# JiawangBian/SC-SfMLearner-Release

Measured on NVIDIA H100. Metric: train-step frames/sec at 256x832 ResNet18 (DispResNet18+PoseResNet18, fwd+bwd+losses+Adam), higher is better.
Workload: dtype tf32x3 (3xTF32 split-accumulate, fp32-level)

## Files before the change

include/scsfm.h:

```cpp
#ifndef SCSFM_H_
#define SCSFM_H_

#include <stddef.h>
#include <stdint.h>

#ifdef __cplusplus
extern "C" {
#endif

#define SCSFM_OK 0
#define SCSFM_ERR_ARG (-1)
#define SCSFM_ERR_CUDA (-2)

#define SCSFM_MAX_JOBS 16

#define SCSFM_WITH_SSIM 1
#define SCSFM_WITH_MASK 2
#define SCSFM_WITH_AUTO_MASK 4
#define SCSFM_DEFER_FINALIZE 0x100
#define SCSFM_PAD_ZEROS 0
#define SCSFM_PAD_BORDER 1

const char* scsfm_last_error(void);
int scsfm_version(void);
long long scsfm_launch_count(void);

typedef struct ScsfmPairJob {
    const float* tgt_img;
    const float* ref_img;
    const float* tgt_depth;
    const float* ref_depth;
    const float* pose;
    float* grad_tgt_depth;
    float* grad_ref_depth;
    float* grad_pose;
    int tgt_shift;
    int ref_shift;
} ScsfmPairJob;

typedef struct ScsfmPairMaps {
    float* warped;
    float* valid;
    float* proj_depth;
    float* comp_depth;
    float* mask;
    float* diff_img;
    float* diff_depth;
} ScsfmPairMaps;

size_t scsfm_pairwise_stats_bytes(int njobs, int B);

int scsfm_pairwise_fwd(const ScsfmPairJob* jobs_host, int njobs, const float* intrinsics, int B, int H, int W,
                       int flags, int padding_mode, void* stats, float* loss_out, const ScsfmPairMaps* maps_host,
                       void* stream);

int scsfm_pairwise_finalize(void* stats, int njobs, float grad_scale, float* loss_out, void* stream);
int scsfm_pairwise_sums_count(int njobs);

int scsfm_pairwise_bwd(const ScsfmPairJob* jobs_host, int njobs, const float* intrinsics, int B, int H, int W,
                       int flags, int padding_mode, void* stats, const float* grad_out, void* stream);

int scsfm_inverse_warp2_fwd(const float* img, const float* depth, const float* ref_depth, const float* pose,
                            const float* intrinsics, int B, int H, int W, int padding_mode, float* warped,
                            float* valid, float* proj_depth, float* comp_depth, void* stream);

int scsfm_inverse_warp2_bwd(const float* img, const float* depth, const float* ref_depth, const float* pose,
                            const float* intrinsics, int B, int H, int W, int padding_mode,
                            const float* grad_warped, const float* grad_proj_depth, const float* grad_comp_depth,
                            float* grad_depth, float* grad_ref_depth, float* grad_pose, void* scratch_12B_doubles,
                            void* stream);

int scsfm_pose_vec2mat(const float* vec, int B, int rotation_mode, float* out, void* stream);

typedef struct ScsfmSmoothJob {
    const float* depth;
    const float* img;
    float* grad_depth;
} ScsfmSmoothJob;

size_t scsfm_smooth_stats_bytes(int njobs, int B);

int scsfm_smooth_fwd(const ScsfmSmoothJob* jobs_host, int njobs, int B, int H, int W, void* stats, float* loss_out,
                     void* stream);
int scsfm_smooth_bwd(const ScsfmSmoothJob* jobs_host, int njobs, int B, int H, int W, void* stats,
                     const float* grad_out, void* stream);


#define SCSFM_PADMODE_ZERO 0
#define SCSFM_PADMODE_REFLECT 1
#define SCSFM_ACT_NONE 0
#define SCSFM_ACT_RELU 1
#define SCSFM_ACT_ELU 2
#define SCSFM_ACT_DISP 3
#define SCSFM_BN_SLOTS 16
#define SCSFM_ROUND_TF32 0x100

typedef struct ScsfmConv {
    const float* in;
    const float* w;
    const float* bias;
    float* out;
    const float* dout;
    float* din;
    const float* addend;
    float* dw;
    float* dbias;
    double* bn_sums;
    int bn_groups;
    int B, Hi, Wi, Cin, Ho, Wo, Cout, kh, kw, stride, pad, pad_mode, act;
    const float* in_lo;
    const float* w_lo;
    const float* dout_lo;
    unsigned tune;
    unsigned long long* debug;
    const float* bn_scale;
    const float* bn_shift;
    float* out_lo;
} ScsfmConv;

#define SCSFM_TUNE_NO_TMA 0x1u
#define SCSFM_TUNE_MT(mt) (((unsigned)(mt) & 3u) << 4)
#define SCSFM_TUNE_TW(l2) (((unsigned)((l2) ? (l2) - 2 : 0) & 3u) << 6)
#define SCSFM_TUNE_BN(bn) (((bn) == 16 ? 1u : (bn) == 32 ? 2u : (bn) == 64 ? 3u : (bn) == 128 ? 4u : 0u) << 8)
#define SCSFM_TUNE_WGRAD(k) (((unsigned)(k) & 3u) << 12)

int scsfm_conv2d_fwd_simt(const ScsfmConv* p, void* stream);
int scsfm_conv2d_dgrad_simt(const ScsfmConv* p, void* stream);
int scsfm_conv2d_wgrad_simt(const ScsfmConv* p, void* stream);

int scsfm_conv2d_fwd_tc(const ScsfmConv* p, void* stream);
int scsfm_conv2d_dgrad_tc(const ScsfmConv* p, void* stream);
int scsfm_conv2d_wgrad_tc(const ScsfmConv* p, void* stream);
#define SCSFM_OPERAND_TF32 0
#define SCSFM_OPERAND_RAW 1
#define SCSFM_OPERAND_LO 2
int scsfm_weight_flip(const float* w, int Cout, int kh, int kw, int Cin, float* wt, int operand, void* stream);
int scsfm_weight_flip_s2(const float* w, int Cout, int kh, int kw, int Cin, int pad, float* wt4, int operand, void* stream);

int scsfm_weight_flip_batched(const long long* table, int n_rows, int total_blocks, void* stream);

int scsfm_head_conv_fwd(const float* in, const float* w, const float* bias, float* out, int B, int H, int W, int C, int act, void* stream);
int scsfm_head_conv_wgrad(const float* in, const float* dpre, float* dw, float* dbias, int B, int H, int W, int C, void* stream);
int scsfm_head_conv_dgrad(const float* dpre, const float* w, float* dpad, int B, int H, int W, int C, void* stream);

int scsfm_nchw_to_nhwc(const float* a, const float* b, int B, int C, int H, int W, float* out, void* stream);
int scsfm_nchw_to_nhwc_pad(const float* a, const float* b, int B, int C, int H, int W, int Cpad, float* out, int operand, void* stream);
int scsfm_pad_channels(const float* src, long long rows, int C, int Cpad, float* dst, int operand, void* stream);
int scsfm_unpad_add(const float* src, long long rows, int C, int Cpad, float* dst, void* stream);
int scsfm_nhwc_to_nchw(const float* in, int B, int C, int H, int W, float* out, void* stream);
int scsfm_stem_dgrad(const float* dy, const float* w, int N, int H, int W, int Cin, float* dimg1, float* dimg2, void* stream);

int scsfm_bn_prepare(const double* sums, int groups, int C, long long count_per_group, const float* gamma,
                     const float* beta, float* running_mean, float* running_var, float momentum, float eps,
                     int training, float* saved, void* stream);
int scsfm_bn_apply(const float* y, const double* sums, const float* gamma, const float* beta, float* running_mean,
                   float* running_var, float momentum, float eps, float* saved, const float* residual, float* z, float* z_lo,
                   long long rows, int C, int groups, int flags, void* stream);
int scsfm_bn_eval_prepare_batched(const long long* table, int n_layers, void* stream);
#define SCSFM_BN_FROZEN 0x200
int scsfm_bn_backward(const float* dz, const float* z, const float* y, const float* saved, const float* gamma,
                      float* dy, float* dy_lo, float* dres, float* dgamma, float* dbeta, long long rows, int C, int groups,
                      int relu, double* work, void* stream);

int scsfm_maxpool_fwd(const float* x, int B, int H, int W, int C, float* y, unsigned char* idx, void* stream);
int scsfm_maxpool_bwd(const float* dy, const unsigned char* idx, int B, int H, int W, int C, float* dx, int accumulate,
                      void* stream);

int scsfm_upcat_fwd(const float* lo, const float* skip, int B, int H, int W, int C1, int C2, float* out, void* stream);
int scsfm_fold_bwd(const float* dpad, int B, int H, int W, int C1, int C2, int upsample, float* d_lo,
                   const float* lo_act, int act, int accumulate, float* d_skip, void* stream);

int scsfm_act_bwd(float* d, const float* out, long long n, int act, void* stream);

int scsfm_spatial_mean_fwd(const float* x, int B, int HW, int C, float scale, float* out, void* stream);
int scsfm_spatial_mean_bwd(const float* dout, int B, int HW, int C, float scale, float* dx, void* stream);

int scsfm_compute_errors(const float* gt, const float* pred, int B, int H, int W, int y1, int y2, int x1, int x2,
                         float max_depth, void* work, float* out, void* stream);

#define SCSFM_EVAL_GT_F32 0
#define SCSFM_EVAL_GT_F64 1
#define SCSFM_EVAL_OUT 12
typedef struct ScsfmEvalDepthImage {
    long long gt_offset;
    int H, W;
    int y1, y2, x1, x2;
} ScsfmEvalDepthImage;
size_t scsfm_eval_depth_workspace_bytes(const ScsfmEvalDepthImage* images_host, int n_img);
int scsfm_eval_depth(const double* pred, int n_img, int h, int w, const void* gt, int gt_dtype, long long gt_elems,
                     const ScsfmEvalDepthImage* images_host, double min_depth, double max_depth, void* workspace,
                     size_t workspace_bytes, double* out, void* stream);

long long scsfm_augment_workspace_ints(int B, int H, int W);
int scsfm_augment_batch(const unsigned char* images, const int* params, int n_img, int B, int H, int W, const float* mean3,
                        const float* std3, float* out, int* workspace, long long workspace_ints, void* stream);

size_t scsfm_resize_bilinear_workspace_bytes(int B, int H, int W, int out_h, int out_w);
int scsfm_resize_bilinear_u8(const unsigned char* in, int B, int H, int W, int out_h, int out_w, unsigned char* out,
                             void* workspace, size_t workspace_bytes, void* stream);

size_t scsfm_velo_depth_workspace_bytes(int B, int Hd, int Wd);
int scsfm_velo_depth(const float* points, const long long* offsets, const long long* offsets_host, const double* P, int B,
                     int Hd, int Wd, float* depth, void* workspace, size_t workspace_bytes, void* stream);

int scsfm_round_tf32(const float* in, float* out, long long n, void* stream);
int scsfm_split_tf32(const float* in, float* lo, long long n, void* stream);

int scsfm_adam_step(float* param, const float* grad, float* exp_avg, float* exp_avg_sq, long long n, float lr,
                    float beta1, float beta2, float eps, float weight_decay, int step, const int* step_dev,
                    float* mirror, int mirror_operand, void* stream);

#ifdef __cplusplus
}
#endif
#endif
```

sc-sfmlearner-release_b200/csrc/conv_tc.cu:

```cuda
#include <stdlib.h>

#include "conv_tc.cuh"

namespace scsfm {

template <int BN, int STAGES, int A_BYTES, int B_BYTES>
__device__ __forceinline__ void gather_consume(float (&acc)[BN / 2], uint8_t* sA, uint8_t* sB, uint64_t* bar_full, uint64_t* bar_empty,
                                               int total, int chain) {
    float part[BN / 2];
#pragma unroll
    for (int i = 0; i < BN / 2; ++i) acc[i] = 0.f;
    for (int it0 = 0; it0 < total; it0 += chain) {
        const int it1 = min(total, it0 + chain);
        for (int it = it0; it < it1; ++it) {
            const int s = it % STAGES;
            tc::mbar_wait(bar_full + s, (it / STAGES) & 1);
            tc::fence_proxy_async();
            const uint32_t a_addr = tc::smem_u32(sA + s * A_BYTES), b_addr = tc::smem_u32(sB + s * B_BYTES);
            tc::reg_fence(part);
            tc::wgmma_fence();
#pragma unroll
            for (int j = 0; j < TBK / 8; ++j)
                tc::wgmma_tf32<BN>(part, tc::make_desc_sw128(a_addr + j * 32), tc::make_desc_sw128(b_addr + j * 32), (it == it0 && j == 0) ? 0u : 1u);
            tc::wgmma_commit();
            tc::wgmma_wait<1>();
            if (it > it0) tc::mbar_arrive(bar_empty + (it - 1) % STAGES);
        }
        tc::wgmma_wait<0>();
        tc::reg_fence(part);
        tc::mbar_arrive(bar_empty + (it1 - 1) % STAGES);
#pragma unroll
        for (int i = 0; i < BN / 2; ++i) acc[i] += part[i];
    }
}

template <int BN, bool STACK = false>
__global__ void __launch_bounds__(FW_THREADS)
conv_fwd_tc_kernel(ScsfmConv p, TcView v, const __grid_constant__ CUtensorMap wmap, const __grid_constant__ CUtensorMap wmap_lo) {
    using Cfg = TcCfg<BN>;
    constexpr int STAGES = Cfg::STAGES;
    extern __shared__ uint8_t smem_raw[];
    uint8_t* smem = reinterpret_cast<uint8_t*>((reinterpret_cast<uintptr_t>(smem_raw) + 1023) & ~uintptr_t(1023));
    uint8_t* sA = smem;
    uint8_t* sB = smem + STAGES * A_STAGE_BYTES;
    uint64_t* bar_full = reinterpret_cast<uint64_t*>(smem + (Cfg::OPERANDS > Cfg::EPI ? Cfg::OPERANDS : Cfg::EPI));
    uint64_t* bar_empty = bar_full + STAGES;

    const int tid = threadIdx.x, warp = tid >> 5, lane = tid & 31;
    const int rows_per_img = v.border ? border_count(p.Ho, p.Wo) : p.Ho * p.Wo;
    const int M = p.B * rows_per_img, N = p.Cout, K = v.kh * v.kw * p.Cin;
    const int m0 = blockIdx.x * GBM, n0 = blockIdx.y * BN;
    const int KB = (K + TBK - 1) / TBK;
    const int npass = STACK ? 2 : 1 + (p.in_lo != nullptr ? 1 : 0) + (p.w_lo != nullptr ? 1 : 0);
    const int chain = npass > 1 ? CHAIN_KB : KB * npass;

    if (tid == 0) {
        for (int s = 0; s < STAGES; ++s) {
            tc::mbar_init(bar_full + s, FW_PWARPS * 32 + 1);
            tc::mbar_init(bar_empty + s, 128);
        }
        tc::fence_barrier_init();
        tc::tma_prefetch_desc(&wmap);
        if (p.w_lo != nullptr) tc::tma_prefetch_desc(&wmap_lo);
    }
    __syncthreads();
    float acc[BN / 2];

    if (warp < FW_PWARPS) {
        constexpr int ROWS = GBM / (FW_PWARPS * 4);
        const int c = tid & 7;
        const int r0 = tid >> 3;
        const int cs = c ^ (r0 & 7);
        const bool reflect = p.pad_mode == PADMODE_REFLECT;
        int hi0[ROWS], wi0[ROWS], rbase[ROWS];
#pragma unroll
        for (int i = 0; i < ROWS; ++i) {
            const int m = m0 + r0 + 16 * i;
            if (m < M) {
                const int b = m / rows_per_img, rem = m - b * rows_per_img;
                int ho, wo;
                if (v.border) border_pixel(rem, p.Ho, p.Wo, ho, wo);
                else { ho = rem / p.Wo; wo = rem - ho * p.Wo; }
                hi0[i] = ho * v.in_stride + v.oy0;
                wi0[i] = wo * v.in_stride + v.ox0;
                rbase[i] = b * p.Hi * p.Wi * p.Cin;
            } else {
                hi0[i] = -(1 << 28);
                wi0[i] = -(1 << 28);
                rbase[i] = 0;
            }
        }
        const uint32_t a_smem = tc::smem_u32(sA) + (uint32_t)(r0 * 128 + cs * 16);
        const uint32_t b_smem = tc::smem_u32(sB);
        int kc, dy, dx, ch;
        int aoff[ROWS];
        uint32_t okm = 0;
        int it = 0;
        for (int q = 0; q < npass; ++q) {
        const int ps = (q + 1) % npass;
        const float* a_base = (ps == 1 && p.in_lo != nullptr) ? p.in_lo : p.in;
        const CUtensorMap* wm = (ps == npass - 1 && ps > 0 && p.w_lo != nullptr) ? &wmap_lo : &wmap;
        kc = 4 * c;
        {
            const int tap = kc / p.Cin;
            ch = kc - tap * p.Cin;
            dy = tap / v.kw;
            dx = tap - dy * v.kw;
        }
        int cur_dy = -1, cur_dx = -1;
        for (int kb = 0; kb < KB; ++kb, ++it) {
            const int s = it % STAGES;
            const uint32_t ph = (it / STAGES) & 1;
            if (lane == 0) tc::mbar_wait(bar_empty + s, ph ^ 1);
            __syncwarp();
            const uint32_t a_st = a_smem + (uint32_t)(s * A_STAGE_BYTES);
            if (tid == 0) {
                tc::mbar_arrive_expect_tx(bar_full + s, (uint32_t)Cfg::B_STAGE_BYTES);
                if (STACK) {
                    tc::tma_load_2d(b_smem + (uint32_t)(s * Cfg::B_STAGE_BYTES), &wmap, kb * TBK, 0, bar_full + s);
                    tc::tma_load_2d(b_smem + (uint32_t)(s * Cfg::B_STAGE_BYTES + (BN / 2) * 128), &wmap_lo, kb * TBK, 0, bar_full + s);
                } else {
                    tc::tma_load_2d(b_smem + (uint32_t)(s * Cfg::B_STAGE_BYTES), wm, kb * TBK, n0, bar_full + s);
                }
            }
            if (dy != cur_dy || dx != cur_dx) {
                cur_dy = dy; cur_dx = dx;
                okm = 0;
#pragma unroll
                for (int i = 0; i < ROWS; ++i) {
                    int hi = hi0[i] + dy, wi = wi0[i] + dx;
                    bool ok;
                    if (reflect) {
                        ok = hi0[i] > -(1 << 27);
                        hi = reflect_index(hi, p.Hi);
                        wi = reflect_index(wi, p.Wi);
                    } else {
                        ok = (unsigned)hi < (unsigned)p.Hi && (unsigned)wi < (unsigned)p.Wi;
                    }
                    aoff[i] = ok ? rbase[i] + (hi * p.Wi + wi) * p.Cin : 0;
                    okm |= (ok ? 1u : 0u) << i;
                }
            }
            const bool kok = kc < K;
#pragma unroll
            for (int i = 0; i < ROWS; ++i) {
                const bool ok = kok && ((okm >> i) & 1u);
                tc::cp_async_16(a_st + i * 2048, a_base + (ok ? aoff[i] + ch : 0), ok ? 16u : 0u);
            }
            tc::cp_async_arrive_noinc(bar_full + s);
            kc += TBK;
            ch += TBK;
            while (ch >= p.Cin) {
                ch -= p.Cin;
                if (++dx == v.kw) { dx = 0; ++dy; }
            }
        }
        }
    } else {
        gather_consume<BN, STAGES, A_STAGE_BYTES, Cfg::B_STAGE_BYTES>(acc, sA, sB, bar_full, bar_empty, KB * npass, chain);
    }

    __syncthreads();
    constexpr int TS = BN + 1;
    float* T = reinterpret_cast<float*>(smem);
    if (warp >= FW_PWARPS) {
        const int t = tid - FW_PWARPS * 32;
        const int r = 16 * (t >> 5) + ((t & 31) >> 2), c = 2 * (t & 3);
#pragma unroll
        for (int i = 0; i < BN / 8; ++i) {
            T[r * TS + 8 * i + c] = acc[4 * i];
            T[r * TS + 8 * i + c + 1] = acc[4 * i + 1];
            T[(r + 8) * TS + 8 * i + c] = acc[4 * i + 2];
            T[(r + 8) * TS + 8 * i + c + 1] = acc[4 * i + 3];
        }
    }
    __syncthreads();
    {
        const int quarter = warp & 1, half = warp >> 1;
        const int m = m0 + quarter * 32 + lane;
        const bool row_ok = m < M;
        size_t out_row = (size_t)m;
        if (row_ok && (v.out_sy != 1 || v.out_sx != 1 || v.border)) {
            const int b = m / rows_per_img, rem = m - b * rows_per_img;
            int ho, wo;
            if (v.border) border_pixel(rem, p.Ho, p.Wo, ho, wo);
            else { ho = rem / p.Wo; wo = rem - ho * p.Wo; }
            out_row = ((size_t)b * v.out_H + (ho * v.out_sy + v.out_oy)) * v.out_W + (wo * v.out_sx + v.out_ox);
        }
        float* stage = T + GBM * TS + warp * (32 * 33);
        constexpr int CREAL = STACK ? BN / 2 : BN;
        constexpr int CW = CREAL < 32 ? CREAL : 32;
        constexpr int NCH = CREAL / CW;
        const float* trow = T + (quarter * 32 + lane) * TS;
#pragma unroll 1
        for (int cc = half; cc < NCH; cc += (FW_PWARPS + 4) / 2) {
            float r[32];
#pragma unroll
            for (int j = 0; j < CW; ++j) r[j] = trow[cc * CW + j];
            if (STACK) {
#pragma unroll
                for (int j = 0; j < CW; ++j) r[j] += trow[BN / 2 + cc * CW + j];
            }
            float v[32];
#pragma unroll
            for (int j = 0; j < CW; ++j) {
                const int n = n0 + cc * CW + j;
                float x = r[j];
                if (row_ok && n < N) {
                    if (p.bias) x += __ldg(p.bias + n);
                    if (p.bn_scale) x = fmaf(x, __ldg(p.bn_scale + n), __ldg(p.bn_shift + n));
                    if (p.addend) x += __ldg(p.addend + out_row * N + n);
                    x = tc_act(x, p.act);
                    if (p.act & ROUND_TF32) x = tf32_round(x);
                } else {
                    x = 0.f;
                }
                v[j] = x;
            }
            if (row_ok) {
                float* o = p.out + out_row * N + n0 + cc * CW;
                if ((N & 3) == 0) {
#pragma unroll
                    for (int j = 0; j < CW; j += 4)
                        if (n0 + cc * CW + j < N) *reinterpret_cast<float4*>(o + j) = make_float4(v[j], v[j + 1], v[j + 2], v[j + 3]);
                } else {
#pragma unroll
                    for (int j = 0; j < CW; ++j)
                        if (n0 + cc * CW + j < N) o[j] = v[j];
                }
                if (p.out_lo != nullptr) {
                    float* ol = p.out_lo + out_row * N + n0 + cc * CW;
#pragma unroll
                    for (int j = 0; j < CW; j += 4)
                        if (n0 + cc * CW + j < N)
                            *reinterpret_cast<float4*>(ol + j) = make_float4(tf32_lo(v[j]), tf32_lo(v[j + 1]), tf32_lo(v[j + 2]), tf32_lo(v[j + 3]));
                }
            }
            if (p.bn_sums != nullptr) {
#pragma unroll
                for (int j = 0; j < CW; ++j) stage[lane * 33 + j] = v[j];
                __syncwarp();
                if (lane < CW) {
                    const int groups = p.bn_groups > 0 ? p.bn_groups : 1;
                    const int rows_per_group = (p.B / groups) * rows_per_img;
                    const int row_base = m0 + quarter * 32;
                    const int n = n0 + cc * CW + lane;
                    int g_cur = row_base / rows_per_group;
                    int next_edge = (g_cur + 1) * rows_per_group - row_base;
                    double s1 = 0.0, s2 = 0.0;
                    for (int rr = 0; rr <= 32; ++rr) {
                        if (rr == 32 || rr == next_edge) {
                            if (n < N && g_cur < groups && (s1 != 0.0 || s2 != 0.0)) {
                                double* d = p.bn_sums + (((size_t)(blockIdx.x % SCSFM_BN_SLOTS) * groups + g_cur) * N + n) * 2;
                                atomicAdd(d, s1);
                                atomicAdd(d + 1, s2);
                            }
                            if (rr == 32) break;
                            s1 = 0.0; s2 = 0.0;
                            ++g_cur;
                            next_edge += rows_per_group;
                        }
                        const double t = (double)stage[rr * 33 + lane];
                        s1 += t;
                        s2 += t * t;
                    }
                }
                __syncwarp();
            }
        }
    }
}

__global__ void weight_flip_kernel(const float* __restrict__ w, int Co, int kh, int kw, int Ci, int jh, int jw, int dy_max,
                                   int dx_max, int step, float* __restrict__ wt, int operand) {
    const long long total = (long long)Co * jh * jw * Ci;
    for (long long i = blockIdx.x * 256LL + threadIdx.x; i < total; i += (long long)gridDim.x * 256) {
        const int o = (int)(i % Co);
        long long t2 = i / Co;
        const int jx = (int)(t2 % jw); t2 /= jw;
        const int jy = (int)(t2 % jh);
        const int c = (int)(t2 / jh);
        const int dy = dy_max - step * jy, dx = dx_max - step * jx;
        wt[i] = tc_operand(__ldg(w + (((size_t)o * kh + dy) * kw + dx) * Ci + c), operand);
    }
}


template <int BN>
struct WgCfg {
    static constexpr int STAGES = 4;
    static constexpr int A_BYTES = GBM * 128;
    static constexpr int B_BYTES = BN * 128;
    static constexpr size_t SMEM = 1024 + (size_t)STAGES * (A_BYTES + B_BYTES) + 256;
};

template <int BN, bool STACK = false>
__global__ void __launch_bounds__(FW_THREADS)
conv_wgrad_tc_kernel(ScsfmConv p, int pix_per_split, int border) {
    using Cfg = WgCfg<BN>;
    constexpr int STAGES = Cfg::STAGES;
    extern __shared__ uint8_t smem_raw[];
    uint8_t* smem = reinterpret_cast<uint8_t*>((reinterpret_cast<uintptr_t>(smem_raw) + 1023) & ~uintptr_t(1023));
    uint8_t* sA = smem;
    uint8_t* sB = smem + STAGES * Cfg::A_BYTES;
    uint64_t* bar_full = reinterpret_cast<uint64_t*>(sB + STAGES * Cfg::B_BYTES);
    uint64_t* bar_empty = bar_full + STAGES;

    const int tid = threadIdx.x, warp = tid >> 5, lane = tid & 31;
    const int HWo = border ? border_count(p.Ho, p.Wo) : p.Ho * p.Wo;
    const int Mtot = p.kh * p.kw * p.Cin, N = p.Cout, npix = p.B * HWo;
    const int m0 = blockIdx.x * GBM, n0 = blockIdx.y * BN;
    const int pix_begin = blockIdx.z * pix_per_split, pix_end = min(npix, pix_begin + pix_per_split);
    const int KB = (pix_end - pix_begin + 31) / 32;
    if (KB <= 0) return;
    const int npass = STACK ? 2 : 1 + (p.in_lo != nullptr ? 1 : 0) + (p.dout_lo != nullptr ? 1 : 0);
    const int chain = npass > 1 ? CHAIN_KB : KB * npass;

    if (tid == 0) {
        for (int s = 0; s < STAGES; ++s) {
            tc::mbar_init(bar_full + s, FW_PWARPS * 32);
            tc::mbar_init(bar_empty + s, 128);
        }
        tc::fence_barrier_init();
    }
    __syncthreads();

    if (warp < FW_PWARPS) {
        constexpr int A_IT = GBM / 4 / FW_PWARPS;
        constexpr int B_IT = BN / 4 / FW_PWARPS;
        const bool reflect = p.pad_mode == PADMODE_REFLECT;
        int a_dy[A_IT], a_dx[A_IT], a_ch[A_IT];
#pragma unroll
        for (int i = 0; i < A_IT; ++i) {
            const int mm = m0 + 4 * (warp + FW_PWARPS * i);
            a_ch[i] = -1;
            a_dy[i] = a_dx[i] = 0;
            if (mm < Mtot) {
                const int tap = mm / p.Cin;
                a_ch[i] = mm - tap * p.Cin;
                a_dy[i] = tap / p.kw - p.pad;
                a_dx[i] = tap - (tap / p.kw) * p.kw - p.pad;
            }
        }
        const uint32_t a_smem = tc::smem_u32(sA), b_smem = tc::smem_u32(sB);
        int fq = 0, fkb = 0, fpx = pix_begin + lane, fb, fho, fwo, frow;
        auto locate = [&]() {
            const int rem = fpx - (fb = fpx / HWo) * HWo;
            if (border) {
                border_pixel(rem, p.Ho, p.Wo, fho, fwo);
                frow = (fb * p.Ho + fho) * p.Wo + fwo;
            } else {
                fho = rem / p.Wo;
                fwo = rem - fho * p.Wo;
                frow = fpx;
            }
        };
        locate();
        auto fetch = [&](float4 (&va)[A_IT], float4 (&vb)[B_IT]) {
            const int ps = (fq + 1) % npass;
            const float* a_base = (ps == 1 && p.in_lo != nullptr) ? p.in_lo : p.in;
            const float* b_main = STACK ? p.dout : ((ps == npass - 1 && ps > 0 && p.dout_lo != nullptr) ? p.dout_lo : p.dout);
            const bool px_ok = fpx < pix_end;
#pragma unroll
            for (int i = 0; i < A_IT; ++i) {
                int hi = fho * p.stride + a_dy[i], wi = fwo * p.stride + a_dx[i];
                bool ok = px_ok && a_ch[i] >= 0;
                if (reflect) { hi = reflect_index(hi, p.Hi); wi = reflect_index(wi, p.Wi); }
                else ok = ok && (unsigned)hi < (unsigned)p.Hi && (unsigned)wi < (unsigned)p.Wi;
                va[i] = ok ? __ldg(reinterpret_cast<const float4*>(a_base + ((size_t)(fb * p.Hi + hi) * p.Wi + wi) * p.Cin + a_ch[i]))
                           : make_float4(0.f, 0.f, 0.f, 0.f);
            }
#pragma unroll
            for (int i = 0; i < B_IT; ++i) {
                const int col = 4 * (warp + FW_PWARPS * i);
                const bool lo_half = STACK && col >= BN / 2;
                const int nn = STACK ? col - (lo_half ? BN / 2 : 0) : n0 + col;
                const bool ok = px_ok && nn < N;
                const float* bb = lo_half ? p.dout_lo : b_main;
                vb[i] = ok ? __ldg(reinterpret_cast<const float4*>(bb + (size_t)frow * N + nn)) : make_float4(0.f, 0.f, 0.f, 0.f);
            }
            if (++fkb == KB) {
                fkb = 0;
                ++fq;
                fpx = pix_begin + lane;
                locate();
            } else if (border) {
                fpx += 32;
                locate();
            } else {
                fpx += 32;
                frow = fpx;
                fwo += 32;
                while (fwo >= p.Wo) { fwo -= p.Wo; if (++fho == p.Ho) { fho = 0; ++fb; } }
            }
        };
        const int total = KB * npass;
        float4 va[A_IT], vb[B_IT];
        fetch(va, vb);
        for (int it = 0; it < total; ++it) {
            float4 na[A_IT], nb[B_IT];
            if (it + 1 < total) fetch(na, nb);
            const int s = it % STAGES;
            tc::mbar_wait(bar_empty + s, ((it / STAGES) & 1) ^ 1);
            const uint32_t a_st = a_smem + (uint32_t)(s * Cfg::A_BYTES), b_st = b_smem + (uint32_t)(s * Cfg::B_BYTES);
#pragma unroll
            for (int i = 0; i < A_IT; ++i) {
                const int r = 4 * (warp + FW_PWARPS * i);
                tc::st_shared_f32(a_st + tc::sw128_offset(r, lane), va[i].x);
                tc::st_shared_f32(a_st + tc::sw128_offset(r + 1, lane), va[i].y);
                tc::st_shared_f32(a_st + tc::sw128_offset(r + 2, lane), va[i].z);
                tc::st_shared_f32(a_st + tc::sw128_offset(r + 3, lane), va[i].w);
            }
#pragma unroll
            for (int i = 0; i < B_IT; ++i) {
                const int r = 4 * (warp + FW_PWARPS * i);
                tc::st_shared_f32(b_st + tc::sw128_offset(r, lane), vb[i].x);
                tc::st_shared_f32(b_st + tc::sw128_offset(r + 1, lane), vb[i].y);
                tc::st_shared_f32(b_st + tc::sw128_offset(r + 2, lane), vb[i].z);
                tc::st_shared_f32(b_st + tc::sw128_offset(r + 3, lane), vb[i].w);
            }
            tc::fence_proxy_async();
            tc::mbar_arrive(bar_full + s);
#pragma unroll
            for (int i = 0; i < A_IT; ++i) va[i] = na[i];
#pragma unroll
            for (int i = 0; i < B_IT; ++i) vb[i] = nb[i];
        }
    } else {
        float acc[BN / 2];
        gather_consume<BN, STAGES, Cfg::A_BYTES, Cfg::B_BYTES>(acc, sA, sB, bar_full, bar_empty, KB * npass, chain);
        const int t = tid - FW_PWARPS * 32;
        const int r = m0 + 16 * (t >> 5) + ((t & 31) >> 2), c = 2 * (t & 3);
#pragma unroll
        for (int i = 0; i < BN / 8; ++i) {
#pragma unroll
            for (int e = 0; e < 4; ++e) {
                const int row = r + 8 * (e >> 1), col = 8 * i + c + (e & 1);
                const int o = STACK ? (col >= BN / 2 ? col - BN / 2 : col) : n0 + col;
                if (row < Mtot && o < N) red_add(p.dw + (size_t)o * Mtot + row, acc[4 * i + e]);
            }
        }
    }
}

CUresult encode_tiled(CUtensorMap* map, CUtensorMapDataType dtype, cuuint32_t rank, void* gaddr, const cuuint64_t* gdim,
                      const cuuint64_t* gstride, const cuuint32_t* box, const cuuint32_t* estr, CUtensorMapInterleave il,
                      CUtensorMapSwizzle sw, CUtensorMapL2promotion l2, CUtensorMapFloatOOBfill oob) {
    using Fn = CUresult (*)(CUtensorMap*, CUtensorMapDataType, cuuint32_t, void*, const cuuint64_t*, const cuuint64_t*, const cuuint32_t*,
                            const cuuint32_t*, CUtensorMapInterleave, CUtensorMapSwizzle, CUtensorMapL2promotion, CUtensorMapFloatOOBfill);
    static Fn fn = nullptr;
    if (fn == nullptr) {
        void* sym = nullptr;
        cudaDriverEntryPointQueryResult qres;
        if (cudaGetDriverEntryPoint("cuTensorMapEncodeTiled", &sym, cudaEnableDefault, &qres) != cudaSuccess || sym == nullptr ||
            qres != cudaDriverEntryPointSuccess)
            return CUDA_ERROR_NOT_FOUND;
        fn = reinterpret_cast<Fn>(sym);
    }
    return fn(map, dtype, rank, gaddr, gdim, gstride, box, estr, il, sw, l2, oob);
}

int launch_bias_grad(const float* dout, int rows, int C, float* dbias, cudaStream_t st);

static int sm_count() {
    static int n = 0;
    if (n == 0) {
        int dev = 0;
        if (cudaGetDevice(&dev) != cudaSuccess || cudaDeviceGetAttribute(&n, cudaDevAttrMultiProcessorCount, dev) != cudaSuccess || n <= 0) n = 132;
    }
    return n;
}

template <int BN, bool STACK = false>
static int launch_wgrad_tc(const ScsfmConv& p, int border, cudaStream_t st) {
    using Cfg = WgCfg<BN>;
    static const cudaError_t attr_rc = cudaFuncSetAttribute(conv_wgrad_tc_kernel<BN, STACK>, cudaFuncAttributeMaxDynamicSharedMemorySize, (int)Cfg::SMEM);
    SCSFM_CHECK_CUDA(attr_rc);
    const int Mtot = p.kh * p.kw * p.Cin, npix = p.B * (border ? border_count(p.Ho, p.Wo) : p.Ho * p.Wo);
    const int mt = (Mtot + GBM - 1) / GBM, nt = STACK ? 1 : (p.Cout + BN - 1) / BN;
    int splits = (sm_count() * 3 + mt * nt - 1) / (mt * nt);
    const int max_splits = (npix + 1023) / 1024;
    if (splits > max_splits) splits = max_splits;
    if (splits < 1) splits = 1;
    const int pps = ((npix + splits - 1) / splits + 31) / 32 * 32;
    dim3 grid(mt, nt, (npix + pps - 1) / pps);
    conv_wgrad_tc_kernel<BN, STACK><<<grid, FW_THREADS, Cfg::SMEM, st>>>(p, pps, border);
    SCSFM_CHECK_LAUNCH();
    return SCSFM_OK;
}

static TcView plain_view(const ScsfmConv& p) {
    return TcView{p.kh, p.kw, -p.pad, -p.pad, p.stride, 1, 0, 1, 0, p.Ho, p.Wo};
}

template <int BN, bool STACK = false>
static int launch_fwd_tc(const ScsfmConv& p, const TcView& v, cudaStream_t st) {
    using Cfg = TcCfg<BN>;
    static const cudaError_t attr_rc = cudaFuncSetAttribute(conv_fwd_tc_kernel<BN, STACK>, cudaFuncAttributeMaxDynamicSharedMemorySize, (int)Cfg::SMEM);
    SCSFM_CHECK_CUDA(attr_rc);
    const int M = p.B * (v.border ? border_count(p.Ho, p.Wo) : p.Ho * p.Wo);
    const int K = v.kh * v.kw * p.Cin;
    CUtensorMap wmap, wmap_lo;
    for (int lo = 0; lo < 2; ++lo) {
        const float* base = lo ? p.w_lo : p.w;
        CUtensorMap& wmap_ = lo ? wmap_lo : wmap;
        if (base == nullptr) { wmap_lo = wmap; continue; }
        const cuuint64_t gdim[2] = {(cuuint64_t)K, (cuuint64_t)p.Cout};
        const cuuint64_t gstride[1] = {(cuuint64_t)K * sizeof(float)};
        const cuuint32_t box[2] = {(cuuint32_t)TBK, (cuuint32_t)(STACK ? BN / 2 : BN)};
        const cuuint32_t estr[2] = {1, 1};
        const CUresult r = encode_tiled(&wmap_, CU_TENSOR_MAP_DATA_TYPE_FLOAT32, 2, const_cast<float*>(base), gdim, gstride, box, estr,
                                                  CU_TENSOR_MAP_INTERLEAVE_NONE, CU_TENSOR_MAP_SWIZZLE_128B, CU_TENSOR_MAP_L2_PROMOTION_L2_256B,
                                                  CU_TENSOR_MAP_FLOAT_OOB_FILL_NONE);
        if (r != CUDA_SUCCESS) {
            set_error("cuTensorMapEncodeTiled(weights %d x %d) failed with CUresult %d", p.Cout, K, (int)r);
            return SCSFM_ERR_CUDA;
        }
    }
    dim3 grid((M + GBM - 1) / GBM, STACK ? 1 : (p.Cout + BN - 1) / BN);
    conv_fwd_tc_kernel<BN, STACK><<<grid, FW_THREADS, Cfg::SMEM, st>>>(p, v, wmap, wmap_lo);
    SCSFM_CHECK_LAUNCH();
    return SCSFM_OK;
}

}

using namespace scsfm;

static int tc_dispatch_gather(const ScsfmConv& p, const TcView& v, cudaStream_t st) {
    const int N = p.Cout;
    if (p.in_lo != nullptr && p.w_lo != nullptr && N <= 64) {
        if (N <= 16) return launch_fwd_tc<32, true>(p, v, st);
        if (N <= 32) return launch_fwd_tc<64, true>(p, v, st);
        return launch_fwd_tc<128, true>(p, v, st);
    }
    if (N <= 16) return launch_fwd_tc<16>(p, v, st);
    if (N <= 32 || N % 64 != 0) return launch_fwd_tc<32>(p, v, st);
    if (N <= 64 || N % 128 != 0) return launch_fwd_tc<64>(p, v, st);
    const int M = p.B * (v.border ? border_count(p.Ho, p.Wo) : p.Ho * p.Wo);
    if (((M + GBM - 1) / GBM) * (N / 128) < sm_count()) return launch_fwd_tc<64>(p, v, st);
    return launch_fwd_tc<128>(p, v, st);
}

static bool s2_prefers_gather(const ScsfmConv& p, const TcView& v) {
    return v.in_stride == 2 && p.in_lo != nullptr && p.Cin >= 512 && p.Ho * p.Wo <= 8 * 26 && !conv_tma_forced(p);
}

static int tc_dispatch(const ScsfmConv& p, const TcView& v, cudaStream_t st) {
    if (p.pad_mode == PADMODE_ZERO && conv_tma_eligible(p, v) && !s2_prefers_gather(p, v)) return launch_conv_tma(p, v, st);
    if (p.pad_mode == PADMODE_REFLECT && v.in_stride == 1 && p.bn_sums == nullptr && p.Ho >= 3 && p.Wo >= 3 &&
        (p.Ho * p.Wo >= 64 * 208 || conv_tma_forced(p)) && conv_tma_eligible(p, v)) {
        ScsfmConv q = p;
        q.pad_mode = PADMODE_ZERO;
        if (int rc = launch_conv_tma(q, v, st)) return rc;
        TcView bv = v;
        bv.border = 1;
        return tc_dispatch_gather(p, bv, st);
    }
    return tc_dispatch_gather(p, v, st);
}

static int check_tc(const ScsfmConv* p, const char* who) {
    SCSFM_CHECK_ARG(p != nullptr && p->in && p->w && p->out, "%s: null tensor", who);
    SCSFM_CHECK_ARG(p->B > 0 && p->Hi > 0 && p->Wi > 0 && p->Cin > 0 && p->Cout > 0 && p->kh > 0 && p->kw > 0 && p->stride > 0 && p->pad >= 0,
                    "%s: bad geometry", who);
    SCSFM_CHECK_ARG((p->Cin & 3) == 0, "%s: the tensor-core kernel needs Cin %% 4 == 0 (got %d); use the CUDA-core kernel", who, p->Cin);
    SCSFM_CHECK_ARG(p->Ho == (p->Hi + 2 * p->pad - p->kh) / p->stride + 1 && p->Wo == (p->Wi + 2 * p->pad - p->kw) / p->stride + 1,
                    "%s: output size does not match geometry", who);
    SCSFM_CHECK_ARG(p->pad_mode != PADMODE_REFLECT || p->pad == 1, "%s: reflect pad must be 1", who);
    if (p->bn_sums) {
        const int g = p->bn_groups > 0 ? p->bn_groups : 1;
        SCSFM_CHECK_ARG(p->B % g == 0, "%s: batch not divisible by the number of BatchNorm groups", who);
    }
    SCSFM_CHECK_ARG((p->bn_scale == nullptr) == (p->bn_shift == nullptr), "%s: bn_scale and bn_shift go together", who);
    SCSFM_CHECK_ARG(p->bn_scale == nullptr || (p->bias == nullptr && p->bn_sums == nullptr),
                    "%s: the eval-mode BatchNorm epilogue excludes bias and bn_sums", who);
    SCSFM_CHECK_ARG(p->out_lo == nullptr || ((p->Cout & 3) == 0 && (reinterpret_cast<uintptr_t>(p->out_lo) & 15) == 0),
                    "%s: out_lo needs Cout %% 4 == 0 and 16-byte alignment", who);
    SCSFM_CHECK_ARG(((reinterpret_cast<uintptr_t>(p->bn_scale) | reinterpret_cast<uintptr_t>(p->bn_shift)) & 7) == 0,
                    "%s: bn_scale / bn_shift must be 8-byte aligned", who);
    return SCSFM_OK;
}

extern "C" int scsfm_conv2d_fwd_tc(const ScsfmConv* p, void* stream) {
    if (int rc = check_tc(p, "conv2d_fwd_tc")) return rc;
    return tc_dispatch(*p, plain_view(*p), (cudaStream_t)stream);
}

extern "C" int scsfm_weight_flip(const float* w, int Cout, int kh, int kw, int Cin, float* wt, int operand, void* stream) {
    SCSFM_CHECK_ARG(w && wt && Cout > 0 && kh > 0 && kw > 0 && Cin > 0 && operand >= 0 && operand <= 2, "weight_flip: bad arguments");
    const long long total = (long long)Cout * kh * kw * Cin;
    int grid = (int)((total + 255) / 256);
    if (grid > sm_count() * 16) grid = sm_count() * 16;
    weight_flip_kernel<<<grid, 256, 0, (cudaStream_t)stream>>>(w, Cout, kh, kw, Cin, kh, kw, kh - 1, kw - 1, 1, wt, operand);
    SCSFM_CHECK_LAUNCH();
    return SCSFM_OK;
}

__global__ void __launch_bounds__(256)
weight_flip_batched_kernel(const long long* __restrict__ table, int n) {
    __shared__ int s_row;
    __shared__ float tile[32][33];
    if (threadIdx.x == 0) {
        int lo = 0, hi = n;
        while (hi - lo > 1) {
            const int mid = (lo + hi) >> 1;
            if (table[mid * 12 + 11] <= (long long)blockIdx.x) lo = mid; else hi = mid;
        }
        s_row = lo;
    }
    __syncthreads();
    const long long* e = table + s_row * 12;
    const float* w = reinterpret_cast<const float*>(e[0]);
    float* wt = reinterpret_cast<float*>(e[1]);
    const int Co = (int)e[2], kh = (int)e[3], kw = (int)e[4], Ci = (int)e[5], jh = (int)e[6], jw = (int)e[7];
    const int dy_max = (int)e[8], dx_max = (int)e[9], step = (int)(e[10] & 0xff), operand = (int)(e[10] >> 8);
    const int tco = (Co + 31) >> 5, tci = (Ci + 31) >> 5;
    int t = (int)((long long)blockIdx.x - e[11]);
    const int to = t % tco; t /= tco;
    const int tc = t % tci; t /= tci;
    const int jy = t / jw, jx = t - jy * jw;
    const int dy = dy_max - step * jy, dx = dx_max - step * jx;
    const int tx = threadIdx.x & 31, ty = threadIdx.x >> 5;
#pragma unroll
    for (int k = 0; k < 4; ++k) {
        const int o = to * 32 + ty + 8 * k, c = tc * 32 + tx;
        if (o < Co && c < Ci) tile[ty + 8 * k][tx] = tc_operand(__ldg(w + (((size_t)o * kh + dy) * kw + dx) * Ci + c), operand);
    }
    __syncthreads();
#pragma unroll
    for (int k = 0; k < 4; ++k) {
        const int c = tc * 32 + ty + 8 * k, o = to * 32 + tx;
        if (c < Ci && o < Co) wt[(((size_t)c * jh + jy) * jw + jx) * Co + o] = tile[tx][ty + 8 * k];
    }
}

extern "C" int scsfm_weight_flip_batched(const long long* table, int n_rows, int total_blocks, void* stream) {
    SCSFM_CHECK_ARG(table != nullptr && n_rows > 0 && total_blocks > 0, "weight_flip_batched: bad arguments");
    weight_flip_batched_kernel<<<total_blocks, 256, 0, (cudaStream_t)stream>>>(table, n_rows);
    SCSFM_CHECK_LAUNCH();
    return SCSFM_OK;
}

extern "C" int scsfm_weight_flip_s2(const float* w, int Cout, int kh, int kw, int Cin, int pad, float* wt4, int operand, void* stream) {
    SCSFM_CHECK_ARG(w && wt4 && Cout > 0 && kh > 0 && kw > 0 && Cin > 0 && pad >= 0 && operand >= 0 && operand <= 2, "weight_flip_s2: bad arguments");
    size_t off = 0;
    for (int py = 0; py < 2; ++py)
        for (int px = 0; px < 2; ++px) {
            int dy_max = kh - 1, dx_max = kw - 1;
            while (dy_max >= 0 && ((py + pad - dy_max) & 1)) --dy_max;
            while (dx_max >= 0 && ((px + pad - dx_max) & 1)) --dx_max;
            const int jh = dy_max < 0 ? 0 : dy_max / 2 + 1, jw = dx_max < 0 ? 0 : dx_max / 2 + 1;
            const long long total = (long long)Cout * jh * jw * Cin;
            if (total > 0) {
                int grid = (int)((total + 255) / 256);
                if (grid > sm_count() * 16) grid = sm_count() * 16;
                weight_flip_kernel<<<grid, 256, 0, (cudaStream_t)stream>>>(w, Cout, kh, kw, Cin, jh, jw, dy_max, dx_max, 2, wt4 + off, operand);
                SCSFM_CHECK_LAUNCH();
            }
            off += (size_t)total;
        }
    return SCSFM_OK;
}

extern "C" int scsfm_conv2d_dgrad_tc(const ScsfmConv* p, void* stream) {
    SCSFM_CHECK_ARG(p != nullptr && p->dout && p->w && p->din, "conv2d_dgrad_tc: null tensor");
    SCSFM_CHECK_ARG(p->stride == 1 || p->stride == 2, "conv2d_dgrad_tc: stride must be 1 or 2");
    SCSFM_CHECK_ARG(p->kh == p->kw && p->kh - 1 - p->pad >= 0, "conv2d_dgrad_tc: square kernels only");
    cudaStream_t st = (cudaStream_t)stream;
    ScsfmConv q = *p;
    q.in = p->dout; q.in_lo = p->dout_lo; q.out = p->din; q.bias = nullptr; q.bn_sums = nullptr; q.act = SCSFM_ACT_NONE;
    q.bn_scale = nullptr; q.bn_shift = nullptr; q.out_lo = nullptr;
    q.dout_lo = nullptr;
    q.Hi = p->Ho; q.Wi = p->Wo; q.Cin = p->Cout;
    q.Cout = p->Cin; q.pad_mode = SCSFM_PADMODE_ZERO;
    if (p->stride == 1) {
        q.Ho = p->Hi; q.Wo = p->Wi;
        q.pad = p->kh - 1 - p->pad;
        if (int rc = check_tc(&q, "conv2d_dgrad_tc")) return rc;
        return tc_dispatch(q, plain_view(q), st);
    }
    SCSFM_CHECK_ARG((q.Cin & 3) == 0, "conv2d_dgrad_tc: needs Cout %% 4 == 0");
    q.stride = 1;
    size_t woff = 0;
    bool covered_all = true;
    for (int py = 0; py < 2; ++py)
        for (int px = 0; px < 2; ++px) {
            int dy_max = p->kh - 1, dx_max = p->kw - 1;
            while (dy_max >= 0 && ((py + p->pad - dy_max) & 1)) --dy_max;
            while (dx_max >= 0 && ((px + p->pad - dx_max) & 1)) --dx_max;
            const int jh = dy_max < 0 ? 0 : dy_max / 2 + 1, jw = dx_max < 0 ? 0 : dx_max / 2 + 1;
            const int Hs = (p->Hi - py + 1) / 2, Ws = (p->Wi - px + 1) / 2;
            if (jh == 0 || jw == 0) { if (Hs > 0 && Ws > 0) covered_all = false; }
            woff += (size_t)p->Cout * jh * jw * p->Cin;
        }
    if (!covered_all) {
        const size_t bytes = (size_t)p->B * p->Hi * p->Wi * p->Cin * sizeof(float);
        if (p->addend) SCSFM_CHECK_CUDA(cudaMemcpyAsync(p->din, p->addend, bytes, cudaMemcpyDeviceToDevice, st));
        else SCSFM_CHECK_CUDA(cudaMemsetAsync(p->din, 0, bytes, st));
    }
    woff = 0;
    for (int py = 0; py < 2; ++py)
        for (int px = 0; px < 2; ++px) {
            int dy_max = p->kh - 1, dx_max = p->kw - 1;
            while (dy_max >= 0 && ((py + p->pad - dy_max) & 1)) --dy_max;
            while (dx_max >= 0 && ((px + p->pad - dx_max) & 1)) --dx_max;
            const int jh = dy_max < 0 ? 0 : dy_max / 2 + 1, jw = dx_max < 0 ? 0 : dx_max / 2 + 1;
            const int Hs = (p->Hi - py + 1) / 2, Ws = (p->Wi - px + 1) / 2;
            const size_t wcount = (size_t)p->Cout * jh * jw * p->Cin;
            if (jh > 0 && jw > 0 && Hs > 0 && Ws > 0) {
                ScsfmConv r = q;
                r.w = p->w + woff;
                r.w_lo = p->w_lo ? p->w_lo + woff : nullptr;
                r.Ho = Hs; r.Wo = Ws; r.kh = jh; r.kw = jw;
                TcView v{jh, jw, (py + p->pad - dy_max) / 2, (px + p->pad - dx_max) / 2, 1, 2, py, 2, px, p->Hi, p->Wi};
                if (int rc = tc_dispatch(r, v, st)) return rc;
            }
            woff += wcount;
        }
    return SCSFM_OK;
}

static int wgrad_gather(const ScsfmConv& p, int border, cudaStream_t st) {
    const bool split = p.in_lo != nullptr && p.dout_lo != nullptr;
    if (split && p.Cout <= 16) return launch_wgrad_tc<32, true>(p, border, st);
    if (split && p.Cout <= 32) return launch_wgrad_tc<64, true>(p, border, st);
    if (split && p.Cout <= 64) return launch_wgrad_tc<128, true>(p, border, st);
    if (p.Cout <= 16) return launch_wgrad_tc<16>(p, border, st);
    if (p.Cout <= 32) return launch_wgrad_tc<32>(p, border, st);
    if (p.Cout <= 64) return launch_wgrad_tc<64>(p, border, st);
    return launch_wgrad_tc<128>(p, border, st);
}

extern "C" int scsfm_conv2d_wgrad_tc(const ScsfmConv* p, void* stream) {
    SCSFM_CHECK_ARG(p != nullptr && p->in && p->dout && p->dw, "conv2d_wgrad_tc: null tensor");
    SCSFM_CHECK_ARG(p->B > 0 && p->Hi > 0 && p->Wi > 0 && p->Cin > 0 && p->Cout > 0 && p->kh > 0 && p->kw > 0 && p->stride > 0 && p->pad >= 0,
                    "conv2d_wgrad_tc: bad geometry");
    SCSFM_CHECK_ARG((p->Cin & 3) == 0 && (p->Cout & 3) == 0, "conv2d_wgrad_tc: needs Cin %% 4 == 0 and Cout %% 4 == 0");
    SCSFM_CHECK_ARG(p->pad_mode != PADMODE_REFLECT || p->pad == 1, "conv2d_wgrad_tc: reflect pad must be 1");
    SCSFM_CHECK_ARG((long long)p->B * p->Ho * p->Wo < (1LL << 31), "conv2d_wgrad_tc: too many pixels");
    cudaStream_t st = (cudaStream_t)stream;
    int rc;
    int kernel = (int)((p->tune >> 12) & 3u);
    if (kernel == 3 && !conv_wgrad_thin_eligible(*p)) kernel = 0;
    if (kernel == 0 && (p->in_lo != nullptr || p->dout_lo != nullptr) && conv_wgrad_thin_eligible(*p)) kernel = 3;
    const bool split = p->in_lo != nullptr && p->dout_lo != nullptr;
    if ((kernel == 0 || kernel == 2) && conv_wgrad_tma_eligible(*p) && (split || (p->in_lo == nullptr && p->dout_lo == nullptr))) {
        if ((rc = launch_conv_wgrad_tma(*p, st))) return rc;
        rc = p->pad_mode == PADMODE_REFLECT ? wgrad_gather(*p, 1, st) : SCSFM_OK;
    } else if (kernel == 3) {
        rc = launch_conv_wgrad_thin(*p, st);
    } else {
        rc = wgrad_gather(*p, 0, st);
    }
    if (rc) return rc;
    if (p->dbias) return launch_bias_grad(p->dout, p->B * p->Ho * p->Wo, p->Cout, p->dbias, st);
    return SCSFM_OK;
}
```

sc-sfmlearner-release_b200/csrc/conv_tc.cuh:

```cuda
#pragma once
#include <cuda.h>

#include "nn_common.cuh"
#include "tc_common.cuh"

namespace scsfm {

constexpr int TBM = 128;
constexpr int GBM = 64;
constexpr int TBK = 32;
constexpr int FW_PWARPS = 4;
constexpr int FW_THREADS = (FW_PWARPS + 4) * 32;
constexpr int A_STAGE_BYTES = GBM * 128;

constexpr int CHAIN_KB = 2;

template <int BN>
struct TcCfg {
    static constexpr int STAGES = 4;
    static constexpr int B_STAGE_BYTES = BN * 128;
    static constexpr size_t OPERANDS = (size_t)STAGES * (A_STAGE_BYTES + B_STAGE_BYTES);
    static constexpr size_t EPI = (size_t)GBM * (BN + 1) * 4 + (size_t)(FW_PWARPS + 4) * 32 * 33 * 4;
    static constexpr size_t SMEM = 1024 + (OPERANDS > EPI ? OPERANDS : EPI) + 256;
};


__device__ __forceinline__ float tc_act(float v, int act) {
    switch (act & 0xff) {
        case ACT_RELU: return fmaxf(v, 0.f);
        case ACT_ELU: return v > 0.f ? v : expm1f(v);
        case ACT_DISP: return 10.0f * (1.0f / (1.0f + expf(-v))) + 0.01f;
        default: return v;
    }
}

struct TcView {
    int kh, kw;
    int oy0, ox0;
    int in_stride;
    int out_sy, out_oy, out_sx, out_ox, out_H, out_W;
    int border;
};

__host__ __device__ __forceinline__ void border_pixel(int j, int Ho, int Wo, int& ho, int& wo) {
    if (j < Wo) { ho = 0; wo = j; }
    else if (j < 2 * Wo) { ho = Ho - 1; wo = j - Wo; }
    else { const int k = j - 2 * Wo; ho = 1 + (k >> 1); wo = (k & 1) ? Wo - 1 : 0; }
}
__host__ __device__ __forceinline__ int border_count(int Ho, int Wo) { return 2 * (Ho + Wo) - 4; }


CUresult encode_tiled(CUtensorMap* map, CUtensorMapDataType dtype, cuuint32_t rank, void* gaddr, const cuuint64_t* gdim,
                      const cuuint64_t* gstride, const cuuint32_t* box, const cuuint32_t* estr, CUtensorMapInterleave il,
                      CUtensorMapSwizzle sw, CUtensorMapL2promotion l2, CUtensorMapFloatOOBfill oob);

bool conv_tma_eligible(const ScsfmConv& p, const TcView& v);
bool conv_tma_forced(const ScsfmConv& p);
int launch_conv_tma(const ScsfmConv& p, const TcView& v, cudaStream_t st);

bool conv_wgrad_tma_eligible(const ScsfmConv& p);
int launch_conv_wgrad_tma(const ScsfmConv& p, cudaStream_t st);

bool conv_wgrad_thin_eligible(const ScsfmConv& p);
int launch_conv_wgrad_thin(const ScsfmConv& p, cudaStream_t st);

}
```

sc-sfmlearner-release_b200/csrc/conv_wgrad_tma.cu:

```cuda
#include <stdlib.h>

#include "conv_tc.cuh"

namespace scsfm {

constexpr int WT_TH = 4, WT_TW = 16;
constexpr int WT_PIX = WT_TH * WT_TW;
constexpr int WT_CK = 64;
constexpr int WT_THREADS = 384;
constexpr int WT_MAX_STAGES = 3;
constexpr int WT_PRODUCER_REGS = 56, WT_CONSUMER_REGS = 224;

template <int BN, bool SPLIT, int KW, int S>
struct WtCfg {
    static constexpr bool STEM = KW == 7;
    static constexpr int PW = S * (WT_TW - 1) + KW;
    static constexpr int PATCH = ((WT_TH * PW * (STEM ? 32 : 128) + 1023) / 1024) * 1024;
    static constexpr int RAW = WT_PIX * 128;
    static constexpr int BT = (WT_PIX / 32) * BN * 128;
    static constexpr int STAGE = 2 * PATCH + (BN / 32) * RAW + (SPLIT ? 2 : 1) * BT;
    static constexpr int STAGES = 2048 + WT_MAX_STAGES * STAGE <= 227 * 1024 ? WT_MAX_STAGES : 2;
    static constexpr size_t SMEM = 1024 + 1024 + (size_t)STAGES * STAGE;
};

struct WtGeom {
    int tiles_x, tiles_y, n_tiles;
    int tiles_per_cta;
    int reflect;
};

__device__ __forceinline__ void setmaxnreg_dec(void) { asm volatile("setmaxnreg.dec.sync.aligned.u32 %0;" ::"n"(WT_PRODUCER_REGS)); }
__device__ __forceinline__ void setmaxnreg_inc(void) { asm volatile("setmaxnreg.inc.sync.aligned.u32 %0;" ::"n"(WT_CONSUMER_REGS)); }

__device__ __forceinline__ uint32_t ld_shared_u32(uint32_t saddr) {
    uint32_t v;
    asm volatile("ld.shared.b32 %0, [%1];" : "=r"(v) : "r"(saddr));
    return v;
}

template <int N>
__device__ __forceinline__ void wgmma_tf32_rs(float (&d)[N / 2], const uint32_t (&a)[4], uint64_t desc_b, uint32_t accumulate);
template <>
__device__ __forceinline__ void wgmma_tf32_rs<32>(float (&d)[16], const uint32_t (&a)[4], uint64_t desc_b, uint32_t accumulate) {
    asm volatile(
        "{\n\t"
        ".reg .pred p;\n\t"
        "setp.ne.b32 p, %21, 0;\n\t"
        "wgmma.mma_async.sync.aligned.m64n32k8.f32.tf32.tf32 {"
        "%0, %1, %2, %3, %4, %5, %6, %7, %8, %9, %10, %11, %12, %13, %14, %15"
        "}, {%16, %17, %18, %19}, %20, p, 1, 1;\n\t"
        "}\n"
        : "+f"(d[0]), "+f"(d[1]), "+f"(d[2]), "+f"(d[3]), "+f"(d[4]), "+f"(d[5]), "+f"(d[6]), "+f"(d[7]),
          "+f"(d[8]), "+f"(d[9]), "+f"(d[10]), "+f"(d[11]), "+f"(d[12]), "+f"(d[13]), "+f"(d[14]), "+f"(d[15])
        : "r"(a[0]), "r"(a[1]), "r"(a[2]), "r"(a[3]), "l"(desc_b), "r"(accumulate));
}
template <>
__device__ __forceinline__ void wgmma_tf32_rs<64>(float (&d)[32], const uint32_t (&a)[4], uint64_t desc_b, uint32_t accumulate) {
    asm volatile(
        "{\n\t"
        ".reg .pred p;\n\t"
        "setp.ne.b32 p, %37, 0;\n\t"
        "wgmma.mma_async.sync.aligned.m64n64k8.f32.tf32.tf32 {"
        "%0, %1, %2, %3, %4, %5, %6, %7, %8, %9, %10, %11, %12, %13, %14, %15, "
        "%16, %17, %18, %19, %20, %21, %22, %23, %24, %25, %26, %27, %28, %29, %30, %31"
        "}, {%32, %33, %34, %35}, %36, p, 1, 1;\n\t"
        "}\n"
        : "+f"(d[0]), "+f"(d[1]), "+f"(d[2]), "+f"(d[3]), "+f"(d[4]), "+f"(d[5]), "+f"(d[6]), "+f"(d[7]),
          "+f"(d[8]), "+f"(d[9]), "+f"(d[10]), "+f"(d[11]), "+f"(d[12]), "+f"(d[13]), "+f"(d[14]), "+f"(d[15]),
          "+f"(d[16]), "+f"(d[17]), "+f"(d[18]), "+f"(d[19]), "+f"(d[20]), "+f"(d[21]), "+f"(d[22]), "+f"(d[23]),
          "+f"(d[24]), "+f"(d[25]), "+f"(d[26]), "+f"(d[27]), "+f"(d[28]), "+f"(d[29]), "+f"(d[30]), "+f"(d[31])
        : "r"(a[0]), "r"(a[1]), "r"(a[2]), "r"(a[3]), "l"(desc_b), "r"(accumulate));
}

template <int BN, bool SPLIT, int KW, int S>
__global__ void __launch_bounds__(WT_THREADS, 1)
conv_wgrad_tma_kernel(ScsfmConv p, WtGeom g, const __grid_constant__ CUtensorMap amap, const __grid_constant__ CUtensorMap amap_odd,
                      const __grid_constant__ CUtensorMap dmap) {
    using Cfg = WtCfg<BN, SPLIT, KW, S>;
    constexpr int PW = Cfg::PW, WT_STAGES = Cfg::STAGES;
    constexpr bool STEM = Cfg::STEM;
    constexpr int NA = STEM ? 1 : KW;
    extern __shared__ uint8_t smem_raw[];
    uint8_t* smem = reinterpret_cast<uint8_t*>((reinterpret_cast<uintptr_t>(smem_raw) + 1023) & ~uintptr_t(1023));
    uint64_t* bar_full = reinterpret_cast<uint64_t*>(smem);
    uint64_t* bar_ready = bar_full + WT_STAGES;
    uint64_t* bar_empty = bar_ready + WT_STAGES;
    const uint32_t ring = tc::smem_u32(smem + 1024);

    const int tid = threadIdx.x, warp = tid >> 5, lane = tid & 31;
    const int dy = blockIdx.x % p.kh, c0 = (blockIdx.x / p.kh) * WT_CK, n0 = blockIdx.y * BN;
    const int t_begin = blockIdx.z * g.tiles_per_cta, t_end = min(g.n_tiles, t_begin + g.tiles_per_cta);
    const int ntile = t_end - t_begin;
    if (ntile <= 0) return;
    const int in_boxes = c0 + 32 < p.Cin ? 2 : 1;

    if (tid == 0) {
        for (int s = 0; s < WT_STAGES; ++s) {
            tc::mbar_init(bar_full + s, 1);
            tc::mbar_init(bar_ready + s, 96);
            tc::mbar_init(bar_empty + s, 256);
        }
        tc::fence_barrier_init();
    }
    __syncthreads();

    auto tile_origin = [&](int t, int& b, int& y0, int& x0) {
        const int tx = t % g.tiles_x;
        t /= g.tiles_x;
        y0 = (t % g.tiles_y) * WT_TH;
        b = t / g.tiles_y;
        x0 = tx * WT_TW;
    };

    if (warp >= 8) {
        setmaxnreg_dec();
        if (warp == 8) {
            if (lane == 0) {
                const int rr = dy - p.pad, par = rr & 1;
                const CUtensorMap* in_map = S == 2 && par ? &amap_odd : &amap;
                const int row_off = S == 2 ? (rr - par) / 2 : rr;
                tc::tma_prefetch_desc(in_map);
                tc::tma_prefetch_desc(&dmap);
                const uint32_t tx_bytes = (uint32_t)(in_boxes * WT_TH * PW * (STEM ? 4 * p.Cin : 128) + (BN / 32) * Cfg::RAW);
                for (int it = 0; it < ntile; ++it) {
                    const int s = it % WT_STAGES;
                    tc::mbar_wait(bar_empty + s, ((it / WT_STAGES) & 1) ^ 1);
                    int b, y0, x0;
                    tile_origin(t_begin + it, b, y0, x0);
                    const uint32_t st = ring + (uint32_t)(s * Cfg::STAGE);
                    tc::mbar_arrive_expect_tx(bar_full + s, tx_bytes);
                    for (int q = 0; q < in_boxes; ++q)
                        tc::tma_load_4d(st + q * Cfg::PATCH, in_map, c0 + 32 * q, S * x0 - p.pad, y0 + row_off, b, bar_full + s);
                    for (int q = 0; q < BN / 32; ++q)
                        tc::tma_load_4d(st + 2 * Cfg::PATCH + q * Cfg::RAW, &dmap, n0 + 32 * q, x0, y0, b, bar_full + s);
                }
            }
            __syncwarp();
        } else {
            const int kcol = S == 2 ? lane : 8 * (lane >> 3) + ((lane & 7) >> 1) + 4 * (lane & 1);
            for (int it = 0; it < ntile; ++it) {
                const int s = it % WT_STAGES;
                tc::mbar_wait(bar_full + s, (it / WT_STAGES) & 1);
                int b, y0, x0;
                tile_origin(t_begin + it, b, y0, x0);
                const uint32_t st = ring + (uint32_t)(s * Cfg::STAGE);
                const uint32_t raw = st + 2 * Cfg::PATCH, bhi = raw + (BN / 32) * Cfg::RAW, blo = bhi + Cfg::BT;
                for (int u = warp - 9; u < (WT_PIX / 32) * (BN / 4); u += 3) {
                    const int kb = u / (BN / 4), oc = u - kb * (BN / 4);
                    const int px = 32 * kb + lane;
                    const int y = y0 + px / WT_TW, x = x0 + px % WT_TW;
                    float4 v;
                    asm volatile("ld.shared.v4.f32 {%0, %1, %2, %3}, [%4];"
                                 : "=f"(v.x), "=f"(v.y), "=f"(v.z), "=f"(v.w)
                                 : "r"(raw + (uint32_t)((oc >> 3) * Cfg::RAW + px * 128 + ((((oc & 7) ^ px) & 7) << 4))));
                    if (g.reflect && (y == 0 || x == 0 || y == p.Ho - 1 || x == p.Wo - 1)) v = make_float4(0.f, 0.f, 0.f, 0.f);
                    const uint32_t o_hi = bhi + (uint32_t)(kb * BN * 128);
                    tc::st_shared_f32(o_hi + tc::sw128_offset(4 * oc, kcol), v.x);
                    tc::st_shared_f32(o_hi + tc::sw128_offset(4 * oc + 1, kcol), v.y);
                    tc::st_shared_f32(o_hi + tc::sw128_offset(4 * oc + 2, kcol), v.z);
                    tc::st_shared_f32(o_hi + tc::sw128_offset(4 * oc + 3, kcol), v.w);
                    if (SPLIT) {
                        const uint32_t o_lo = blo + (uint32_t)(kb * BN * 128);
                        tc::st_shared_f32(o_lo + tc::sw128_offset(4 * oc, kcol), tf32_lo(v.x));
                        tc::st_shared_f32(o_lo + tc::sw128_offset(4 * oc + 1, kcol), tf32_lo(v.y));
                        tc::st_shared_f32(o_lo + tc::sw128_offset(4 * oc + 2, kcol), tf32_lo(v.z));
                        tc::st_shared_f32(o_lo + tc::sw128_offset(4 * oc + 3, kcol), tf32_lo(v.w));
                    }
                }
                tc::fence_proxy_async();
                tc::mbar_arrive(bar_ready + s);
            }
        }
        return;
    }

    setmaxnreg_inc();
    const int wg = warp >> 2, w = warp & 3;
    const int gq = lane >> 2, tq = lane & 3;
    const int cc = 16 * (w & 1) + gq;
    const int m_rows = STEM ? 7 * p.Cin : p.Cin;
    const bool w_ok = c0 + 16 * w < m_rows;
    float acc[NA][BN / 2];
#pragma unroll
    for (int dx = 0; dx < NA; ++dx)
#pragma unroll
        for (int i = 0; i < BN / 2; ++i) acc[dx][i] = 0.f;
    float part[BN / 2];
    for (int it = 0; it < ntile; ++it) {
        const int s = it % WT_STAGES;
        const uint32_t ph = (it / WT_STAGES) & 1;
        tc::mbar_wait(bar_full + s, ph);
        tc::mbar_wait(bar_ready + s, ph);
        const uint32_t st = ring + (uint32_t)(s * Cfg::STAGE);
        const uint32_t patch = st + (uint32_t)((w >> 1) * Cfg::PATCH);
        const uint32_t bhi = st + 2 * Cfg::PATCH + (BN / 32) * Cfg::RAW, blo = bhi + Cfg::BT;
#pragma unroll
        for (int dx = 0; dx < NA; ++dx) {
#pragma unroll
            for (int h = 0; h < (SPLIT ? 2 : 1); ++h) {
                constexpr int NS = SPLIT ? 2 : 4;
                uint32_t ahi[NS][4], alo[NS][4];
#pragma unroll
                for (int j = 0; j < NS; ++j) {
                    const int sl = 4 * wg + NS * h + j;
                    const int pbase = (sl >> 1) * PW + S * (8 * (sl & 1)) + dx + 2 * tq;
#pragma unroll
                    for (int e = 0; e < 4; ++e) {
                        if (STEM) {
                            const int m = 16 * w + gq + 8 * (e & 1), px = 8 * (sl & 1) + tq + 4 * (e >> 1);
                            ahi[j][e] = m < m_rows ? ld_shared_u32(st + (uint32_t)((((sl >> 1) * PW + 2 * px) * p.Cin + m) * 4)) : 0u;
                        } else {
                            const int pp = pbase + (S == 2 ? 8 : 1) * (e >> 1), ch = cc + 8 * (e & 1);
                            ahi[j][e] = w_ok ? ld_shared_u32(patch + tc::sw128_offset(pp, ch)) : 0u;
                        }
                        if (SPLIT) alo[j][e] = __float_as_uint(tf32_lo(__uint_as_float(ahi[j][e])));
                    }
                }
                if (SPLIT) {
                    tc::reg_fence(part);
                    tc::wgmma_fence();
#pragma unroll
                    for (int j = 0; j < NS; ++j) {
                        const int sl = 4 * wg + NS * h + j;
                        const uint32_t boff = (uint32_t)((sl >> 2) * BN * 128 + (sl & 3) * 32);
                        wgmma_tf32_rs<BN>(part, alo[j], tc::make_desc_sw128(bhi + boff), j == 0 ? 0u : 1u);
                        wgmma_tf32_rs<BN>(part, ahi[j], tc::make_desc_sw128(blo + boff), 1u);
                    }
#pragma unroll
                    for (int j = 0; j < NS; ++j) {
                        const int sl = 4 * wg + NS * h + j;
                        const uint32_t boff = (uint32_t)((sl >> 2) * BN * 128 + (sl & 3) * 32);
                        wgmma_tf32_rs<BN>(part, ahi[j], tc::make_desc_sw128(bhi + boff), 1u);
                    }
                    tc::wgmma_commit();
                    tc::wgmma_wait<0>();
                    tc::reg_fence(part);
#pragma unroll
                    for (int i = 0; i < BN / 2; ++i) acc[dx][i] += part[i];
                } else {
                    tc::reg_fence(acc[dx]);
                    tc::wgmma_fence();
#pragma unroll
                    for (int j = 0; j < NS; ++j) {
                        const int sl = 4 * wg + j;
                        const uint32_t boff = (uint32_t)((sl >> 2) * BN * 128 + (sl & 3) * 32);
                        wgmma_tf32_rs<BN>(acc[dx], ahi[j], tc::make_desc_sw128(bhi + boff), 1u);
                    }
                    tc::wgmma_commit();
                    tc::wgmma_wait<0>();
                    tc::reg_fence(acc[dx]);
                }
            }
        }
        tc::mbar_arrive(bar_empty + s);
    }
    const int kwr = p.kw;
    if (STEM) {
#pragma unroll
        for (int i = 0; i < BN / 8; ++i) {
#pragma unroll
            for (int e = 0; e < 4; ++e) {
                const int m = 16 * w + gq + 8 * (e >> 1), o = n0 + 8 * i + 2 * tq + (e & 1);
                if (m < m_rows && o < p.Cout) red_add(p.dw + ((size_t)o * p.kh + dy) * m_rows + m, acc[0][4 * i + e]);
            }
        }
        return;
    }
#pragma unroll
    for (int dx = 0; dx < NA; ++dx) {
        if (dx >= kwr) break;
#pragma unroll
        for (int i = 0; i < BN / 8; ++i) {
#pragma unroll
            for (int e = 0; e < 4; ++e) {
                const int c = c0 + 16 * w + gq + 8 * (e >> 1), o = n0 + 8 * i + 2 * tq + (e & 1);
                if (c < p.Cin && o < p.Cout) red_add(p.dw + (((size_t)o * p.kh + dy) * kwr + dx) * p.Cin + c, acc[dx][4 * i + e]);
            }
        }
    }
}

bool conv_wgrad_tma_eligible(const ScsfmConv& p) {
    if (p.tune & SCSFM_TUNE_NO_TMA) return false;
    const bool stem = p.stride == 2 && p.kh == 7 && p.kw == 7 && (p.Cin == 4 || p.Cin == 8);
    if (!stem && ((p.stride != 1 && p.stride != 2) || p.kh > 3 || p.kw > 3)) return false;
    if ((p.Cin & 3) != 0 || (p.Cout & 3) != 0) return false;
    if (p.pad_mode == PADMODE_REFLECT && (p.stride != 1 || p.Ho < 3 || p.Wo < 3)) return false;
    if (p.stride == 2 && p.Hi < 2) return false;
    return true;
}

static int sm_count() {
    static int n = 0;
    if (n == 0) {
        int dev = 0;
        if (cudaGetDevice(&dev) != cudaSuccess || cudaDeviceGetAttribute(&n, cudaDevAttrMultiProcessorCount, dev) != cudaSuccess || n <= 0) n = 132;
    }
    return n;
}

static int encode_nhwc(CUtensorMap* map, const float* base, int B, int H, int W, int C, int box_w, int box_h, int rows, int row_step,
                       int box_c = TBK, CUtensorMapSwizzle sw = CU_TENSOR_MAP_SWIZZLE_128B) {
    const cuuint64_t gdim[4] = {(cuuint64_t)C, (cuuint64_t)W, (cuuint64_t)rows, (cuuint64_t)B};
    const cuuint64_t gstride[3] = {(cuuint64_t)C * 4, (cuuint64_t)row_step * W * C * 4, (cuuint64_t)H * W * C * 4};
    const cuuint32_t box[4] = {(cuuint32_t)box_c, (cuuint32_t)box_w, (cuuint32_t)box_h, 1};
    const cuuint32_t estr[4] = {1, 1, 1, 1};
    const CUresult r = encode_tiled(map, CU_TENSOR_MAP_DATA_TYPE_FLOAT32, 4, const_cast<float*>(base), gdim, gstride, box, estr,
                                    CU_TENSOR_MAP_INTERLEAVE_NONE, sw, CU_TENSOR_MAP_L2_PROMOTION_L2_256B,
                                    CU_TENSOR_MAP_FLOAT_OOB_FILL_NONE);
    if (r != CUDA_SUCCESS) {
        set_error("cuTensorMapEncodeTiled(%d x %d x %d x %d) failed with CUresult %d", B, H, W, C, (int)r);
        return SCSFM_ERR_CUDA;
    }
    return SCSFM_OK;
}

template <int BN, bool SPLIT, int KW, int S>
static int launch_wgrad_tma_cfg(const ScsfmConv& p, cudaStream_t st) {
    using Cfg = WtCfg<BN, SPLIT, KW, S>;
    static const cudaError_t attr_rc =
        cudaFuncSetAttribute(conv_wgrad_tma_kernel<BN, SPLIT, KW, S>, cudaFuncAttributeMaxDynamicSharedMemorySize, (int)Cfg::SMEM);
    SCSFM_CHECK_CUDA(attr_rc);
    CUtensorMap amap, amap_odd, dmap;
    if (S == 1) {
        if (int rc = encode_nhwc(&amap, p.in, p.B, p.Hi, p.Wi, p.Cin, Cfg::PW, WT_TH, p.Hi, 1)) return rc;
        amap_odd = amap;
    } else {
        const int box_c = Cfg::STEM ? p.Cin : TBK;
        const CUtensorMapSwizzle sw = Cfg::STEM ? CU_TENSOR_MAP_SWIZZLE_NONE : CU_TENSOR_MAP_SWIZZLE_128B;
        if (int rc = encode_nhwc(&amap, p.in, p.B, p.Hi, p.Wi, p.Cin, Cfg::PW, WT_TH, (p.Hi + 1) / 2, 2, box_c, sw)) return rc;
        if (int rc = encode_nhwc(&amap_odd, p.in + (size_t)p.Wi * p.Cin, p.B, p.Hi, p.Wi, p.Cin, Cfg::PW, WT_TH, p.Hi / 2, 2, box_c, sw))
            return rc;
    }
    if (int rc = encode_nhwc(&dmap, p.dout, p.B, p.Ho, p.Wo, p.Cout, WT_TW, WT_TH, p.Ho, 1)) return rc;
    WtGeom g;
    g.tiles_x = (p.Wo + WT_TW - 1) / WT_TW;
    g.tiles_y = (p.Ho + WT_TH - 1) / WT_TH;
    g.n_tiles = g.tiles_x * g.tiles_y * p.B;
    g.reflect = p.pad_mode == PADMODE_REFLECT;
    const int mt = ((p.Cin + WT_CK - 1) / WT_CK) * p.kh, nt = (p.Cout + BN - 1) / BN;
    int splits = sm_count() / (mt * nt);
    const int max_splits = (g.n_tiles + 7) / 8;
    if (splits > max_splits) splits = max_splits;
    if (splits < 1) splits = 1;
    g.tiles_per_cta = (g.n_tiles + splits - 1) / splits;
    dim3 grid(mt, nt, (g.n_tiles + g.tiles_per_cta - 1) / g.tiles_per_cta);
    conv_wgrad_tma_kernel<BN, SPLIT, KW, S><<<grid, WT_THREADS, Cfg::SMEM, st>>>(p, g, amap, amap_odd, dmap);
    SCSFM_CHECK_LAUNCH();
    return SCSFM_OK;
}

template <int BN, bool SPLIT>
static int launch_wgrad_tma_bn(const ScsfmConv& p, cudaStream_t st) {
    if (p.stride == 2 && p.kw == 7) return launch_wgrad_tma_cfg<BN, SPLIT, 7, 2>(p, st);
    if (p.stride == 2) return p.kw == 1 ? launch_wgrad_tma_cfg<BN, SPLIT, 1, 2>(p, st) : launch_wgrad_tma_cfg<BN, SPLIT, 3, 2>(p, st);
    return p.kw == 1 ? launch_wgrad_tma_cfg<BN, SPLIT, 1, 1>(p, st) : launch_wgrad_tma_cfg<BN, SPLIT, 3, 1>(p, st);
}

int launch_conv_wgrad_tma(const ScsfmConv& p, cudaStream_t st) {
    const bool split = p.in_lo != nullptr && p.dout_lo != nullptr;
    const unsigned bn_knob = (p.tune >> 8) & 7u;
    const bool bn32 = bn_knob == 2 || (bn_knob != 3 && p.Cout <= 32);
    if (bn32) return split ? launch_wgrad_tma_bn<32, true>(p, st) : launch_wgrad_tma_bn<32, false>(p, st);
    return split ? launch_wgrad_tma_bn<64, true>(p, st) : launch_wgrad_tma_bn<64, false>(p, st);
}

}
```

sc-sfmlearner-release_b200/csrc/tc_common.cuh:

```cuda
#pragma once
#include <cuda_runtime.h>
#include <stdint.h>

namespace scsfm {
namespace tc {

__device__ __forceinline__ uint32_t smem_u32(const void* p) { return (uint32_t)__cvta_generic_to_shared(p); }

__device__ __forceinline__ void st_shared_v4(uint32_t saddr, const float4& v) {
    asm volatile("st.shared.v4.f32 [%0], {%1, %2, %3, %4};" ::"r"(saddr), "f"(v.x), "f"(v.y), "f"(v.z), "f"(v.w) : "memory");
}

__device__ __forceinline__ void st_shared_f32(uint32_t saddr, float v) {
    asm volatile("st.shared.f32 [%0], %1;" ::"r"(saddr), "f"(v) : "memory");
}

__device__ __forceinline__ void cp_async_16(uint32_t saddr, const void* gptr, uint32_t src_bytes) {
    asm volatile("cp.async.cg.shared.global [%0], [%1], 16, %2;" ::"r"(saddr), "l"(gptr), "r"(src_bytes) : "memory");
}
__device__ __forceinline__ void cp_async_arrive_noinc(uint64_t* bar) {
    asm volatile("cp.async.mbarrier.arrive.noinc.shared::cta.b64 [%0];" ::"r"(smem_u32(bar)) : "memory");
}

__device__ __forceinline__ void mbar_init(uint64_t* bar, uint32_t count) {
    asm volatile("mbarrier.init.shared::cta.b64 [%0], %1;" ::"r"(smem_u32(bar)), "r"(count) : "memory");
}
__device__ __forceinline__ void mbar_arrive(uint64_t* bar) {
    asm volatile("mbarrier.arrive.shared::cta.b64 _, [%0];" ::"r"(smem_u32(bar)) : "memory");
}
__device__ __forceinline__ void mbar_wait(uint64_t* bar, uint32_t parity) {
    asm volatile(
        "{\n\t"
        ".reg .pred p;\n\t"
        "LAB_WAIT:\n\t"
        "mbarrier.try_wait.parity.shared::cta.b64 p, [%0], %1;\n\t"
        "@p bra LAB_DONE;\n\t"
        "bra LAB_WAIT;\n\t"
        "LAB_DONE:\n\t"
        "}\n" ::"r"(smem_u32(bar)),
        "r"(parity)
        : "memory");
}
__device__ __forceinline__ void fence_barrier_init() { asm volatile("fence.mbarrier_init.release.cluster;" ::: "memory"); }
__device__ __forceinline__ void fence_proxy_async() { asm volatile("fence.proxy.async.shared::cta;" ::: "memory"); }

__device__ __forceinline__ void mbar_arrive_expect_tx(uint64_t* bar, uint32_t bytes) {
    asm volatile("mbarrier.arrive.expect_tx.shared::cta.b64 _, [%0], %1;" ::"r"(smem_u32(bar)), "r"(bytes) : "memory");
}
__device__ __forceinline__ void tma_load_2d(uint32_t smem_dst, const void* tensor_map, int c0, int c1, uint64_t* bar) {
    asm volatile("cp.async.bulk.tensor.2d.shared::cluster.global.tile.mbarrier::complete_tx::bytes [%0], [%1, {%2, %3}], [%4];"
                 ::"r"(smem_dst), "l"(reinterpret_cast<uint64_t>(tensor_map)), "r"(c0), "r"(c1), "r"(smem_u32(bar))
                 : "memory");
}
__device__ __forceinline__ void tma_load_4d(uint32_t smem_dst, const void* tensor_map, int c0, int c1, int c2, int c3, uint64_t* bar) {
    asm volatile("cp.async.bulk.tensor.4d.shared::cluster.global.tile.mbarrier::complete_tx::bytes [%0], [%1, {%2, %3, %4, %5}], [%6];"
                 ::"r"(smem_dst), "l"(reinterpret_cast<uint64_t>(tensor_map)), "r"(c0), "r"(c1), "r"(c2), "r"(c3), "r"(smem_u32(bar))
                 : "memory");
}
__device__ __forceinline__ void tma_prefetch_desc(const void* tensor_map) {
    asm volatile("prefetch.tensormap [%0];" ::"l"(reinterpret_cast<uint64_t>(tensor_map)) : "memory");
}

template <int R>
__device__ __forceinline__ void setmaxnreg_dec() { asm volatile("setmaxnreg.dec.sync.aligned.u32 %0;" ::"n"(R)); }
template <int R>
__device__ __forceinline__ void setmaxnreg_inc() { asm volatile("setmaxnreg.inc.sync.aligned.u32 %0;" ::"n"(R)); }

__device__ __forceinline__ void wgmma_fence() { asm volatile("wgmma.fence.sync.aligned;" ::: "memory"); }
__device__ __forceinline__ void wgmma_commit() { asm volatile("wgmma.commit_group.sync.aligned;" ::: "memory"); }
template <int N>
__device__ __forceinline__ void wgmma_wait() { asm volatile("wgmma.wait_group.sync.aligned %0;" ::"n"(N) : "memory"); }
template <int R>
__device__ __forceinline__ void reg_fence(float (&d)[R]) {
#pragma unroll
    for (int i = 0; i < R; ++i) asm volatile("" : "+f"(d[i])::"memory");
}

template <int N>
__device__ __forceinline__ void wgmma_tf32(float (&d)[N / 2], uint64_t desc_a, uint64_t desc_b, uint32_t accumulate);
template <>
__device__ __forceinline__ void wgmma_tf32<16>(float (&d)[8], uint64_t desc_a, uint64_t desc_b, uint32_t accumulate) {
    asm volatile(
        "{\n\t"
        ".reg .pred p;\n\t"
        "setp.ne.b32 p, %10, 0;\n\t"
        "wgmma.mma_async.sync.aligned.m64n16k8.f32.tf32.tf32 {"
        "%0, %1, %2, %3, %4, %5, %6, %7"
        "}, %8, %9, p, 1, 1;\n\t"
        "}\n"
        : "+f"(d[0]), "+f"(d[1]), "+f"(d[2]), "+f"(d[3]), "+f"(d[4]), "+f"(d[5]), "+f"(d[6]), "+f"(d[7])
        : "l"(desc_a), "l"(desc_b), "r"(accumulate));
}
template <>
__device__ __forceinline__ void wgmma_tf32<32>(float (&d)[16], uint64_t desc_a, uint64_t desc_b, uint32_t accumulate) {
    asm volatile(
        "{\n\t"
        ".reg .pred p;\n\t"
        "setp.ne.b32 p, %18, 0;\n\t"
        "wgmma.mma_async.sync.aligned.m64n32k8.f32.tf32.tf32 {"
        "%0, %1, %2, %3, %4, %5, %6, %7, %8, %9, %10, %11, %12, %13, %14, %15"
        "}, %16, %17, p, 1, 1;\n\t"
        "}\n"
        : "+f"(d[0]), "+f"(d[1]), "+f"(d[2]), "+f"(d[3]), "+f"(d[4]), "+f"(d[5]), "+f"(d[6]), "+f"(d[7]),
          "+f"(d[8]), "+f"(d[9]), "+f"(d[10]), "+f"(d[11]), "+f"(d[12]), "+f"(d[13]), "+f"(d[14]), "+f"(d[15])
        : "l"(desc_a), "l"(desc_b), "r"(accumulate));
}
template <>
__device__ __forceinline__ void wgmma_tf32<64>(float (&d)[32], uint64_t desc_a, uint64_t desc_b, uint32_t accumulate) {
    asm volatile(
        "{\n\t"
        ".reg .pred p;\n\t"
        "setp.ne.b32 p, %34, 0;\n\t"
        "wgmma.mma_async.sync.aligned.m64n64k8.f32.tf32.tf32 {"
        "%0, %1, %2, %3, %4, %5, %6, %7, %8, %9, %10, %11, %12, %13, %14, %15, "
        "%16, %17, %18, %19, %20, %21, %22, %23, %24, %25, %26, %27, %28, %29, %30, %31"
        "}, %32, %33, p, 1, 1;\n\t"
        "}\n"
        : "+f"(d[0]), "+f"(d[1]), "+f"(d[2]), "+f"(d[3]), "+f"(d[4]), "+f"(d[5]), "+f"(d[6]), "+f"(d[7]),
          "+f"(d[8]), "+f"(d[9]), "+f"(d[10]), "+f"(d[11]), "+f"(d[12]), "+f"(d[13]), "+f"(d[14]), "+f"(d[15]),
          "+f"(d[16]), "+f"(d[17]), "+f"(d[18]), "+f"(d[19]), "+f"(d[20]), "+f"(d[21]), "+f"(d[22]), "+f"(d[23]),
          "+f"(d[24]), "+f"(d[25]), "+f"(d[26]), "+f"(d[27]), "+f"(d[28]), "+f"(d[29]), "+f"(d[30]), "+f"(d[31])
        : "l"(desc_a), "l"(desc_b), "r"(accumulate));
}
template <>
__device__ __forceinline__ void wgmma_tf32<128>(float (&d)[64], uint64_t desc_a, uint64_t desc_b, uint32_t accumulate) {
    asm volatile(
        "{\n\t"
        ".reg .pred p;\n\t"
        "setp.ne.b32 p, %66, 0;\n\t"
        "wgmma.mma_async.sync.aligned.m64n128k8.f32.tf32.tf32 {"
        "%0, %1, %2, %3, %4, %5, %6, %7, %8, %9, %10, %11, %12, %13, %14, %15, "
        "%16, %17, %18, %19, %20, %21, %22, %23, %24, %25, %26, %27, %28, %29, %30, %31, "
        "%32, %33, %34, %35, %36, %37, %38, %39, %40, %41, %42, %43, %44, %45, %46, %47, "
        "%48, %49, %50, %51, %52, %53, %54, %55, %56, %57, %58, %59, %60, %61, %62, %63"
        "}, %64, %65, p, 1, 1;\n\t"
        "}\n"
        : "+f"(d[0]), "+f"(d[1]), "+f"(d[2]), "+f"(d[3]), "+f"(d[4]), "+f"(d[5]), "+f"(d[6]), "+f"(d[7]),
          "+f"(d[8]), "+f"(d[9]), "+f"(d[10]), "+f"(d[11]), "+f"(d[12]), "+f"(d[13]), "+f"(d[14]), "+f"(d[15]),
          "+f"(d[16]), "+f"(d[17]), "+f"(d[18]), "+f"(d[19]), "+f"(d[20]), "+f"(d[21]), "+f"(d[22]), "+f"(d[23]),
          "+f"(d[24]), "+f"(d[25]), "+f"(d[26]), "+f"(d[27]), "+f"(d[28]), "+f"(d[29]), "+f"(d[30]), "+f"(d[31]),
          "+f"(d[32]), "+f"(d[33]), "+f"(d[34]), "+f"(d[35]), "+f"(d[36]), "+f"(d[37]), "+f"(d[38]), "+f"(d[39]),
          "+f"(d[40]), "+f"(d[41]), "+f"(d[42]), "+f"(d[43]), "+f"(d[44]), "+f"(d[45]), "+f"(d[46]), "+f"(d[47]),
          "+f"(d[48]), "+f"(d[49]), "+f"(d[50]), "+f"(d[51]), "+f"(d[52]), "+f"(d[53]), "+f"(d[54]), "+f"(d[55]),
          "+f"(d[56]), "+f"(d[57]), "+f"(d[58]), "+f"(d[59]), "+f"(d[60]), "+f"(d[61]), "+f"(d[62]), "+f"(d[63])
        : "l"(desc_a), "l"(desc_b), "r"(accumulate));
}

__device__ __forceinline__ uint64_t make_desc_sw128(uint32_t saddr) {
    uint64_t d = 0;
    d |= (uint64_t)((saddr >> 4) & 0x3FFF);
    d |= (uint64_t)1 << 16;
    d |= (uint64_t)(1024 >> 4) << 32;
    d |= (uint64_t)1 << 62;
    return d;
}

__host__ __device__ __forceinline__ uint32_t sw128_offset(int r, int k) {
    return (uint32_t)(r * 128 + ((((k >> 2) ^ r) & 7) << 4) + ((k & 3) << 2));
}

}
}
```

sc-sfmlearner-release_b200/scsfm/nets.py:

```python
import collections
import math

import torch
import torch.nn as nn

from . import nnops as O

BN_EPS, BN_MOMENTUM = 1e-5, 0.1
STAGE_BLOCKS = {18: (2, 2, 2, 2), 34: (3, 4, 6, 3), 50: (3, 4, 6, 3), 101: (3, 4, 23, 3), 152: (3, 8, 36, 3)}


class ConvParams(nn.Module):
    def __init__(self, cin, cout, k, bias, init):
        super().__init__()
        w = torch.empty(cout, cin, k, k)
        if init == "kaiming_fan_out":
            nn.init.kaiming_normal_(w, mode="fan_out", nonlinearity="relu")
        else:
            nn.init.kaiming_uniform_(w, a=math.sqrt(5))
        self.weight = nn.Parameter(w.contiguous(memory_format=torch.channels_last))
        if bias:
            bound = 1.0 / math.sqrt(cin * k * k)
            self.bias = nn.Parameter(torch.empty(cout).uniform_(-bound, bound))
        else:
            self.bias = None
        self.k = k

    def w_khwc(self):
        return self.weight.permute(0, 2, 3, 1)

    def w_op(self, cx):
        tc = getattr(self, "_tc_view", None)
        return tc if (tc is not None and cx.mode == "tf32") else self.w_khwc()

    def w_lo(self, cx):
        return self._tc_view if cx.split else None


class BNParams(nn.Module):
    def __init__(self, c):
        super().__init__()
        self.weight = nn.Parameter(torch.ones(c))
        self.bias = nn.Parameter(torch.zeros(c))
        self.register_buffer("running_mean", torch.zeros(c))
        self.register_buffer("running_var", torch.ones(c))
        self.register_buffer("num_batches_tracked", torch.tensor(0, dtype=torch.long))


class LinearParams(nn.Module):

    def __init__(self, cin, cout):
        super().__init__()
        bound = 1.0 / math.sqrt(cin)
        w = torch.empty(cout, cin)
        nn.init.kaiming_uniform_(w, a=math.sqrt(5))
        self.weight = nn.Parameter(w)
        self.bias = nn.Parameter(torch.empty(cout).uniform_(-bound, bound))


class Block(nn.Module):

    def __init__(self, cin, width, stride, bottleneck):
        super().__init__()
        self.bottleneck, self.stride = bottleneck, stride
        cout = width * (4 if bottleneck else 1)
        if bottleneck:
            self.conv1, self.bn1 = ConvParams(cin, width, 1, False, "kaiming_fan_out"), BNParams(width)
            self.conv2, self.bn2 = ConvParams(width, width, 3, False, "kaiming_fan_out"), BNParams(width)
            self.conv3, self.bn3 = ConvParams(width, cout, 1, False, "kaiming_fan_out"), BNParams(cout)
        else:
            self.conv1, self.bn1 = ConvParams(cin, width, 3, False, "kaiming_fan_out"), BNParams(width)
            self.conv2, self.bn2 = ConvParams(width, width, 3, False, "kaiming_fan_out"), BNParams(width)
        self.downsample = None
        if stride != 1 or cin != cout:
            self.downsample = nn.Sequential(ConvParams(cin, cout, 1, False, "kaiming_fan_out"), BNParams(cout))
        self.cout = cout

    def units(self):
        if self.bottleneck:
            main = [(self.conv1, self.bn1, 1, 0), (self.conv2, self.bn2, self.stride, 1), (self.conv3, self.bn3, 1, 0)]
        else:
            main = [(self.conv1, self.bn1, self.stride, 1), (self.conv2, self.bn2, 1, 1)]
        ds = None if self.downsample is None else (self.downsample[0], self.downsample[1], self.stride, 0)
        return main, ds


class Trunk(nn.Module):
    def __init__(self, num_layers, in_ch):
        super().__init__()
        bott = num_layers >= 50
        self.conv1, self.bn1 = ConvParams(in_ch, 64, 7, False, "kaiming_fan_out"), BNParams(64)
        cin = 64
        for i, (n, width) in enumerate(zip(STAGE_BLOCKS[num_layers], (64, 128, 256, 512))):
            blocks = []
            for j in range(n):
                blk = Block(cin, width, 2 if (j == 0 and i > 0) else 1, bott)
                blocks.append(blk)
                cin = blk.cout
            setattr(self, "layer%d" % (i + 1), nn.Sequential(*blocks))
        self.fc = LinearParams(cin, 1000)


class ResnetEncoder(nn.Module):
    def __init__(self, num_layers, pretrained, num_input_images=1):
        super().__init__()
        if num_layers not in STAGE_BLOCKS:
            raise ValueError("{} is not a valid number of resnet layers".format(num_layers))
        self.num_ch_enc = [64, 64, 128, 256, 512] if num_layers <= 34 else [64, 256, 512, 1024, 2048]
        self.encoder = Trunk(num_layers, 3 * num_input_images)
        if pretrained:
            self.load_imagenet(num_layers, num_input_images)

    def load_imagenet(self, num_layers, num_input_images):
        import glob
        import os
        dirs = [os.environ.get("SCSFM_PRETRAINED_DIR", ""), os.path.join(torch.hub.get_dir(), "checkpoints")]
        hits = [f for d in dirs if d for f in sorted(glob.glob(os.path.join(d, "resnet%d-*.pth" % num_layers)))]
        if not hits:
            raise FileNotFoundError("no local ImageNet checkpoint resnet%d-*.pth in %s (no network access: put the torchvision "
                                    "file there, or use pretrained=False / --with-pretrain 0)" % (num_layers, [d for d in dirs if d]))
        sd = torch.load(hits[0], map_location="cpu")
        if num_input_images > 1:
            sd["conv1.weight"] = torch.cat([sd["conv1.weight"]] * num_input_images, 1) / num_input_images
        own = self.encoder.state_dict()
        for k, v in sd.items():
            if k in own and own[k].shape == v.shape:
                own[k].copy_(v)


class _ReflConv(nn.Module):
    def __init__(self, cin, cout):
        super().__init__()
        self.conv = ConvParams(int(cin), int(cout), 3, True, "default")


class _ReflConvELU(nn.Module):
    def __init__(self, cin, cout):
        super().__init__()
        self.conv = _ReflConv(cin, cout)


class DepthDecoder(nn.Module):
    def __init__(self, num_ch_enc):
        super().__init__()
        dec = [16, 32, 64, 128, 256]
        mods, self.idx = [], {}
        for i in range(4, -1, -1):
            cin = num_ch_enc[-1] if i == 4 else dec[i + 1]
            self.idx[("up", i, 0)] = len(mods)
            mods.append(_ReflConvELU(cin, dec[i]))
            cin = dec[i] + (num_ch_enc[i - 1] if i > 0 else 0)
            self.idx[("up", i, 1)] = len(mods)
            mods.append(_ReflConvELU(cin, dec[i]))
        for s in range(4):
            self.idx[("disp", s)] = len(mods)
            mods.append(_ReflConv(dec[s], 1))
        self.decoder = nn.ModuleList(mods)

    def up(self, i, j):
        return self.decoder[self.idx[("up", i, j)]].conv.conv

    def disp(self, s):
        return self.decoder[self.idx[("disp", s)]].conv


class PoseDecoder(nn.Module):
    def __init__(self, num_ch_enc):
        super().__init__()
        self.net = nn.ModuleList([ConvParams(num_ch_enc[-1], 256, 1, True, "default"),
                                  ConvParams(256, 256, 3, True, "default"), ConvParams(256, 256, 3, True, "default"),
                                  ConvParams(256, 6, 1, True, "default")])


POSE_HEAD = ((0, O.ACT_RELU), (1, O.ACT_RELU), (1, O.ACT_RELU), (0, O.ACT_NONE))


def _pose_act(cx, k):
    act = POSE_HEAD[k][1]
    return act | cx.rnd() if k + 1 < len(POSE_HEAD) else act


class ArenaNet(nn.Module):

    def __init__(self):
        super().__init__()
        self._flat = None
        self._flat_grad = None
        self._views = []
        self._hook = None
        self._pending = 0
        self.grads_ready_callback = None
        self.ctx = O.ConvCtx("fp32")

    @property
    def conv_mode(self):
        return self.ctx.mode

    def set_conv_mode(self, mode):
        if mode != self.ctx.mode:
            pool, ws = self.ctx.sums_pool, self.ctx.wgrad_stream
            self.ctx = O.ConvCtx(mode)
            self.ctx.sums_pool, self.ctx.wgrad_stream = pool, ws
            self._tf32_version = None
        return self

    def _arena_ok(self):
        if self._flat is None:
            return False
        p0 = next(self.parameters())
        if p0.device != self._flat.device:
            return False
        off = 0
        for p in self.parameters():
            if p.data_ptr() != self._flat.data_ptr() + 4 * off:
                return False
            off += O.aligned64(p.numel())
        return True

    def ensure_arena(self):
        if self._arena_ok():
            return
        params = list(self.parameters())
        dev = params[0].device
        if dev.type != "cuda":
            raise RuntimeError("the networks run on CUDA only (no CPU fallback): move the module with .to('cuda')")
        n = sum(O.aligned64(p.numel()) for p in params)
        flat = torch.zeros(n, device=dev, dtype=torch.float32)
        gflat = torch.zeros(n, device=dev, dtype=torch.float32)
        self._flat_tf32 = torch.zeros_like(flat)
        convs = {id(m.weight): m for m in self.modules() if isinstance(m, ConvParams)}
        views, off = [], 0
        for p in params:
            cnt = p.numel()
            if p.dim() == 4:
                O_, I_, kh, kw = p.shape
                dst = flat[off:off + cnt].view(O_, kh, kw, I_).permute(0, 3, 1, 2)
                gv = gflat[off:off + cnt].view(O_, kh, kw, I_).permute(0, 3, 1, 2)
                convs[id(p)]._tc_view = self._flat_tf32[off:off + cnt].view(O_, kh, kw, I_)
            else:
                dst = flat[off:off + cnt].view(p.shape)
                gv = gflat[off:off + cnt].view(p.shape)
            dst.copy_(p.data)
            p.data = dst
            p.grad = gv
            views.append((p, gv))
            off += O.aligned64(cnt)
        self._flat, self._flat_grad, self._views = flat, gflat, views
        self._hook = torch.zeros(1, device=dev, requires_grad=True)
        bns = [m for m in self.modules() if isinstance(m, BNParams)]
        if bns:
            nbt = torch.stack([m.num_batches_tracked.to(dev) for m in bns])
            for i, m in enumerate(bns):
                m.num_batches_tracked = nbt[i]
            for m in self.modules():
                if isinstance(m, ResnetEncoder):
                    m._nbt = nbt
        self._tf32_version = None
        self.ctx.invalidate()

    trust_adam_mirror = False
    _tf32_version = None

    def _versions(self):
        return (self._flat._version, sum(p._version for p, _ in self._views))

    def refresh_operand_weights(self):
        cx = self.ctx
        if cx.tc:
            if not (self.trust_adam_mirror and self._tf32_version == self._versions()):
                if cx.split:
                    O.split_tf32(self._flat, self._flat_tf32)
                else:
                    O.round_tf32(self._flat, self._flat_tf32)
                self._tf32_version = self._versions()
            cx.refresh_flips(self._flat.device)

    def _fused_eval(self):
        return not self.training and not torch.is_grad_enabled()

    def _call(self, inputs, groups=None):
        G = groups or 1
        self.ensure_arena()
        if self._fused_eval():
            outs = self._forward_impl(G, *inputs, fused=True)[1]
        else:
            if torch.is_grad_enabled():
                self._pending += 1
            outs = _NetCall.apply(self, self._hook, G, *inputs)
        if groups is None:
            return outs
        B = inputs[0].shape[0] // G
        return [[o[g * B:(g + 1) * B] for o in outs] for g in range(G)]

    def bn_eval_coeffs(self):
        bns = [m for m in self.modules() if isinstance(m, BNParams)]
        tab = getattr(self, "_bn_eval", None)
        if tab is None or tab.key != O.BnEvalTable.key_of(bns):
            tab = self._bn_eval = O.BnEvalTable(bns, BN_EPS)
        tab.prepare()
        return {id(bn): c for bn, c in zip(bns, tab.coeffs)}

    def _attach_grads(self):
        if self._views and self._views[0][0].grad is None:
            self._flat_grad.zero_()
        for p, gv in self._views:
            if p.grad is not gv:
                p.grad = gv

    def zero_grad(self, set_to_none=False):
        if self._flat_grad is not None:
            self._flat_grad.zero_()
            for p, gv in self._views:
                p.grad = gv
        else:
            super().zero_grad(set_to_none=set_to_none)

    def flat_params(self):
        self.ensure_arena()
        return self._flat

    def flat_grads(self):
        self.ensure_arena()
        return self._flat_grad

    @staticmethod
    def g(p):
        return p.grad.permute(0, 2, 3, 1) if p.dim() == 4 else p.grad


class BackwardPlan:

    def __init__(self, training=True, params=True, dimg=(False, False)):
        self.bn = 0 if training else O.BN_FROZEN
        self.params = params
        self.dimg = tuple(bool(n) for n in dimg)


TRAIN_PLAN = BackwardPlan()


class _NetCall(torch.autograd.Function):
    @staticmethod
    def forward(ctx, net, hook, groups, *inputs):
        rec, outs = net._forward_impl(groups, *inputs)
        ctx.net, ctx.rec = net, rec
        ctx.set_materialize_grads(False)
        return tuple(outs)

    @staticmethod
    def backward(ctx, *grads):
        net = ctx.net
        need = ctx.needs_input_grad[3:]
        plan = BackwardPlan(ctx.rec["training"], any(p.requires_grad for p, _ in net._views), need)
        dimgs = [None] * len(need)
        if plan.params or any(need):
            if plan.params:
                net._attach_grads()
            dimgs = net._backward_impl(ctx.rec, [None if g is None else g.contiguous() for g in grads], plan)
            net.ctx.join_wgrad()
        ctx.rec = None
        net._pending -= 1
        if net._pending == 0 and net.grads_ready_callback is not None:
            net.grads_ready_callback(net)
        return (None, None, None) + tuple(dimgs)


class _SumsPool:

    def __init__(self):
        self.buf, self.cursor, self.need = {}, 0, 0

    def begin(self, device):
        self.need = max(self.need, self.cursor)
        buf = self.buf.get(device)
        if buf is None or buf.numel() < self.need:
            buf = self.buf[device] = torch.zeros(max(self.need, 1 << 16), device=device, dtype=torch.float64)
        elif self.cursor:
            buf[:self.cursor].zero_()
        self.cursor = 0

    def take(self, n, device):
        n = (n + 31) // 32 * 32
        buf = self.buf.get(device)
        start, self.cursor = self.cursor, self.cursor + n
        if buf is None or self.cursor > buf.numel():
            return torch.zeros(n, device=device, dtype=torch.float64)
        return buf[start:start + n]


def _pool(cx):
    if cx.sums_pool is None:
        cx.sums_pool = _SumsPool()
    return cx.sums_pool


class _Forward:

    def __init__(self, net, groups, fused):
        self.cx, self.training, self.groups = net.ctx, net.training, groups
        self.coeffs = net.bn_eval_coeffs() if fused else None

    @property
    def fused(self):
        return self.coeffs is not None


_Unit = collections.namedtuple("_Unit", "x y z saved")


def _conv_bn(f, x, unit, relu, residual=None, with_lo=False, w=None):
    conv, bn, stride, pad = unit
    cx = f.cx
    w, w_lo = (conv.w_op(cx), conv.w_lo(cx)) if w is None else w
    if f.fused:
        sc, sh = f.coeffs[id(bn)]
        z = cx.conv_fwd(x, w, None, stride, pad, O.PAD_ZERO, (O.ACT_RELU if relu else O.ACT_NONE) | cx.rnd(), None, 1, w_lo,
                        bn_scale=sc, bn_shift=sh, addend=residual, with_lo=with_lo and cx.split)
        return z, None
    G = f.groups
    sums = _pool(cx).take(O.BN_SLOTS * G * conv.weight.shape[0] * 2, x.device) if f.training else None
    y = cx.conv_fwd(x, w, None, stride, pad, O.PAD_ZERO, O.ACT_NONE, sums, G, w_lo)
    z, saved = O.bn_apply(y, sums, bn.weight, bn.bias, bn.running_mean, bn.running_var, BN_MOMENTUM, BN_EPS, residual,
                          (1 if relu else 0) | cx.rnd(), G, cx.split)
    return z, _Unit(x, y, z if relu else None, saved)


def _bn_param_grads(bn, plan):
    return (bn.weight.grad, bn.bias.grad) if plan.params else (None, None)


def _conv_bn_bwd(cx, dz, unit, r, relu, want_dres, addend, groups, plan):
    conv, bn, stride, pad = unit
    dy, dres = O.bn_backward(dz, r.z, r.y, r.saved, *_bn_param_grads(bn, plan), (1 if relu else 0) | cx.rnd() | plan.bn, want_dres,
                             groups, cx.split)
    if plan.params:
        cx.conv_wgrad(r.x, dy, ArenaNet.g(conv.weight), None, stride, pad, O.PAD_ZERO)
    return cx.conv_dgrad(dy, conv.w_op(cx), r.x.shape, stride, pad, addend), dres


def block_forward(f, blk, x):
    main, ds = blk.units()
    h, recs = x, []
    for unit in main[:-1]:
        h, r = _conv_bn(f, h, unit, True, with_lo=True)
        recs.append(r)
    sc, ds_rec = (x, None) if ds is None else _conv_bn(f, x, ds, False)
    out, r = _conv_bn(f, h, main[-1], True, sc, with_lo=True)
    return out, None if f.fused else (recs + [r], ds_rec)


def block_backward(cx, blk, rec, d_out, d_skip, groups, plan):
    main, ds = blk.units()
    recs, ds_rec = rec
    d, dres = _conv_bn_bwd(cx, d_out, main[-1], recs[-1], True, True, None, groups, plan)
    for k in range(len(main) - 2, 0, -1):
        d, _ = _conv_bn_bwd(cx, d, main[k], recs[k], True, False, None, groups, plan)
    if ds is not None:
        d_sc, _ = _conv_bn_bwd(cx, dres, ds, ds_rec, False, False, d_skip, groups, plan)
    else:
        assert d_skip is None, "skip-connection gradient at a block without downsample"
        d_sc = dres
    dx, _ = _conv_bn_bwd(cx, d, main[0], recs[0], True, False, d_sc, groups, plan)
    return dx


def _stem_operands(cx, conv, imgs):
    if not cx.tc:
        return O.nchw_to_nhwc(imgs[0], imgs[1] if len(imgs) > 1 else None), conv.w_op(cx), conv.w_lo(cx)
    cpad = 4 * len(imgs)
    x_nhwc = O.nchw_to_nhwc_pad(imgs[0], imgs[1] if len(imgs) > 1 else None, cpad, cx.operand)
    w = O.pad_channels(conv.w_khwc(), cpad, cx.operand)
    w_lo = O.pad_channels(conv.w_khwc(), cpad, O.OPERAND_LO) if cx.split else None
    return x_nhwc, w, w_lo


def encoder_forward(f, enc, imgs):
    t = enc.encoder
    G = f.groups
    if f.training:
        _pool(f.cx).begin(imgs[0].device)
        nbt = getattr(enc, "_nbt", None)
        if nbt is not None:
            nbt.add_(G)
        else:
            for m in enc.modules():
                if isinstance(m, BNParams):
                    m.num_batches_tracked += G
    x_nhwc, w0, w0_lo = _stem_operands(f.cx, t.conv1, imgs)
    f0, stem = _conv_bn(f, x_nhwc, (t.conv1, t.bn1, 2, 3), True, w=(w0, w0_lo))
    del x_nhwc, w0, w0_lo
    x, pool_idx = O.maxpool_fwd(f0)
    feats, blocks = [f0], []
    for li in range(1, 5):
        for blk in getattr(t, "layer%d" % li):
            x, r = block_forward(f, blk, x)
            blocks.append((blk, r))
        feats.append(x)
    return None if f.fused else {"G": G, "stem": stem, "pool_idx": pool_idx, "blocks": blocks}, feats


def encoder_backward(cx, enc, rec, d_feats, plan=TRAIN_PLAN):
    t = enc.encoder
    blocks, G = rec["blocks"], rec["G"]
    ends, k = {}, 0
    for li in range(1, 5):
        k += len(getattr(t, "layer%d" % li))
        ends[k - 1] = li
    d = d_feats[4]
    for bi in range(len(blocks) - 1, -1, -1):
        blk, r = blocks[bi]
        extra = None
        if bi - 1 in ends and d_feats[ends[bi - 1]] is not None:
            extra = d_feats[ends[bi - 1]]
        d = block_backward(cx, blk, r, d, extra, G, plan)
    stem = rec["stem"]
    f0, x = stem.z, stem.x
    if d_feats[0] is not None:
        d_f0 = d_feats[0]
        O.maxpool_bwd(d, rec["pool_idx"], f0.shape, d_f0, True)
    else:
        d_f0 = torch.empty_like(f0)
        O.maxpool_bwd(d, rec["pool_idx"], f0.shape, d_f0, False)
    dy, _ = O.bn_backward(d_f0, f0, stem.y, stem.saved, *_bn_param_grads(t.bn1, plan), 1 | cx.rnd() | plan.bn, False, G,
                          cx.split and plan.params)
    if plan.params:
        if x.shape[-1] != t.conv1.weight.shape[1]:
            dw = torch.zeros(t.conv1.weight.shape[0], t.conv1.k, t.conv1.k, x.shape[-1], device=x.device, dtype=torch.float32)
            cx.conv_wgrad(x, dy, dw, None, 2, 3, O.PAD_ZERO)
            with cx.on_wgrad_stream([dw]):
                O.unpad_add_(ArenaNet.g(t.conv1.weight), dw)
        else:
            cx.conv_wgrad(x, dy, ArenaNet.g(t.conv1.weight), None, 2, 3, O.PAD_ZERO)
    if not any(plan.dimg):
        return [None] * len(plan.dimg)
    return O.stem_dgrad(dy, t.conv1.w_khwc(), x.shape[1], x.shape[2], plan.dimg)


class DispResNet(ArenaNet):

    def __init__(self, num_layers=18, pretrained=True):
        super().__init__()
        self.encoder = ResnetEncoder(num_layers=num_layers, pretrained=pretrained, num_input_images=1)
        self.decoder = DepthDecoder(self.encoder.num_ch_enc)

    def init_weights(self):
        pass

    def forward(self, x):
        outs = self._call((x,))
        return list(outs) if self.training else outs[0]

    def forward_multi(self, images):
        per = self._call((torch.cat(list(images), 0),), len(images))
        return per if self.training else [p[0] for p in per]

    def _forward_impl(self, groups, x, fused=False):
        from . import lib as L
        x = L.dev_f32(x, "DispResNet input")
        self.refresh_operand_weights()
        training = self.training
        cx = self.ctx
        enc_rec, feats = encoder_forward(_Forward(self, groups, fused), self.encoder, (x,))
        dec = self.decoder
        rec = {"enc": enc_rec, "stages": {}, "training": training}
        cur = feats[4]
        disps = {}
        for i in range(4, -1, -1):
            c0 = dec.up(i, 0)
            a = cx.conv_fwd(cur, c0.w_op(cx), c0.bias, 1, 1, O.PAD_REFLECT, O.ACT_ELU | cx.rnd(), None, 1, c0.w_lo(cx))
            cat = O.upcat_fwd(a, feats[i - 1] if i > 0 else None)
            c1 = dec.up(i, 1)
            b = cx.conv_fwd(cat, c1.w_op(cx), c1.bias, 1, 1, O.PAD_REFLECT, O.ACT_ELU | cx.rnd(), None, 1, c1.w_lo(cx),
                            with_lo=fused and cx.split and i > 0)
            if fused:
                if i > 0:
                    feats[i - 1] = None
            else:
                rec["stages"][i] = {"in0": cur, "a": a, "cat": cat, "b": b}
            del a, cat
            cur = b
            if i < 4 and (training or i == 0):
                dc = dec.disp(i)
                disps[i] = O.head_fwd(cur, dc.w_khwc(), dc.bias, O.ACT_DISP)
        rec["disps"] = disps
        order = [0, 1, 2, 3] if training else [0]
        rec["order"] = order
        return None if fused else rec, [disps[s].view(disps[s].shape[0], 1, disps[s].shape[1], disps[s].shape[2]) for s in order]

    def _backward_impl(self, rec, grads, plan=TRAIN_PLAN):
        dec = self.decoder
        g = ArenaNet.g
        cx = self.ctx
        d_disp = {s: gr for s, gr in zip(rec["order"], grads) if gr is not None}
        d_feats = [None] * 5
        d_b = None
        pending = None
        for i in range(0, 5):
            st = rec["stages"][i]
            b = st["b"]
            have = pending is not None
            d_b = pending
            if i in d_disp:
                dc = dec.disp(i)
                disp = rec["disps"][i]
                dpre = O.act_bwd_(d_disp[i].reshape(disp.shape).clone(), disp, O.ACT_DISP)
                if plan.params:
                    O.head_wgrad(b, dpre, g(dc.weight), dc.bias.grad)
                dpad = O.head_dgrad(dpre, dc.w_khwc(), b.shape)
                if not have:
                    d_b = torch.empty_like(b)
                O.fold_plain(dpad, d_b, b, O.ACT_ELU | cx.rnd(), accumulate=have)
            elif have:
                O.act_bwd_(d_b, b, O.ACT_ELU | cx.rnd())
            else:
                continue
            c1 = dec.up(i, 1)
            if plan.params:
                cx.conv_wgrad(st["cat"], d_b, g(c1.weight), c1.bias.grad, 1, 1, O.PAD_REFLECT)
            dpad = cx.conv_dgrad(d_b, c1.w_op(cx), st["cat"].shape, 1, 1, None, padded_input=True)
            d_a, d_skip = O.fold_upcat(dpad, st["a"].shape[-1], st["a"], O.ACT_ELU | cx.rnd())
            if i > 0:
                d_feats[i - 1] = d_skip
            c0 = dec.up(i, 0)
            if plan.params:
                cx.conv_wgrad(st["in0"], d_a, g(c0.weight), c0.bias.grad, 1, 1, O.PAD_REFLECT)
            dpad = cx.conv_dgrad(d_a, c0.w_op(cx), st["in0"].shape, 1, 1, None, padded_input=True)
            d_in = torch.empty_like(st["in0"])
            O.fold_plain(dpad, d_in, None, O.ACT_NONE, accumulate=False)
            if i < 4:
                pending = d_in
            else:
                d_feats[4] = d_in
        return encoder_backward(cx, self.encoder, rec["enc"], d_feats, plan)


class PoseResNet(ArenaNet):

    def __init__(self, num_layers=18, pretrained=True):
        super().__init__()
        self.encoder = ResnetEncoder(num_layers=num_layers, pretrained=pretrained, num_input_images=2)
        self.decoder = PoseDecoder(self.encoder.num_ch_enc)

    def init_weights(self):
        pass

    def forward(self, img1, img2):
        return self._call((img1, img2))[0]

    def forward_multi(self, pairs):
        per = self._call((torch.cat([a for a, _ in pairs], 0), torch.cat([b for _, b in pairs], 0)), len(pairs))
        return [p[0] for p in per]

    def _forward_impl(self, groups, img1, img2, fused=False):
        from . import lib as L
        img1, img2 = L.dev_f32(img1, "PoseResNet input"), L.dev_f32(img2, "PoseResNet input")
        self.refresh_operand_weights()
        cx = self.ctx
        enc_rec, feats = encoder_forward(_Forward(self, groups, fused), self.encoder, (img1, img2))
        x = feats[4]
        del feats
        head = None if fused else [x]
        for k, (pad, _) in enumerate(POSE_HEAD):
            conv = self.decoder.net[k]
            x = cx.conv_fwd(x, conv.w_op(cx), conv.bias, 1, pad, O.PAD_ZERO, _pose_act(cx, k), None, 1, conv.w_lo(cx),
                            with_lo=fused and cx.split and k < 2)
            if head is not None:
                head.append(x)
        rec = None if fused else {"enc": enc_rec, "head": head, "training": self.training}
        return rec, [O.spatial_mean_fwd(x, 0.01)]

    def _backward_impl(self, rec, grads, plan=TRAIN_PLAN):
        cx = self.ctx
        head = rec["head"]
        d = O.spatial_mean_bwd(grads[0], head[-1].shape, 0.01)
        for k in range(len(POSE_HEAD) - 1, -1, -1):
            conv, pad, inp = self.decoder.net[k], POSE_HEAD[k][0], head[k]
            if plan.params:
                cx.conv_wgrad(inp, d, ArenaNet.g(conv.weight), conv.bias.grad, 1, pad, O.PAD_ZERO)
            d = cx.conv_dgrad(d, conv.w_op(cx), inp.shape, 1, pad)
            if k > 0:
                O.act_bwd_(d, inp, _pose_act(cx, k - 1))
        return encoder_backward(cx, self.encoder, rec["enc"], [None, None, None, None, d], plan)


class ArenaAdam:

    def __init__(self, nets, lr=1e-4, betas=(0.9, 0.999), eps=1e-8, weight_decay=0.0):
        self.nets = list(nets)
        self.lr, self.betas, self.eps, self.weight_decay = lr, betas, eps, weight_decay
        self.state = {}
        self._step = None

    @property
    def step_count(self):
        return 0 if self._step is None else int(self._step.item())

    def zero_grad(self, set_to_none=False):
        for n in self.nets:
            n.ensure_arena()
            n.zero_grad()

    def _ensure_state(self):
        for n in self.nets:
            n.ensure_arena()
            key = id(n)
            if key not in self.state or self.state[key][2] is not n._flat:
                self.state[key] = (torch.zeros_like(n._flat), torch.zeros_like(n._flat), n._flat)
        if self._step is None:
            self._step = torch.zeros(1, device=self.nets[0]._flat.device, dtype=torch.int32)

    def step(self):
        self._ensure_state()
        self._step += 1
        for n in self.nets:
            n._pending = 0
            m, v, _ = self.state[id(n)]
            mirror = n._flat_tf32 if n.ctx.tc else None
            O.adam_step(n._flat, n._flat_grad, m, v, self.lr, self.betas[0], self.betas[1], self.eps, self.weight_decay,
                        0, self._step, mirror, O.OPERAND_LO if n.ctx.split else O.OPERAND_TF32)
            n._tf32_version = n._versions() if mirror is not None else None

    def snapshot(self):
        self._ensure_state()
        snap = {"step": self._step.clone(), "nets": []}
        for n in self.nets:
            m, v, _ = self.state[id(n)]
            snap["nets"].append((n._flat.clone(), m.clone(), v.clone(), {k: b.clone() for k, b in n.named_buffers()}))
        return snap

    def restore(self, snap):
        self._step.copy_(snap["step"])
        for n, (flat, m0, v0, bufs) in zip(self.nets, snap["nets"]):
            m, v, _ = self.state[id(n)]
            n._flat.copy_(flat); m.copy_(m0); v.copy_(v0)
            for k, b in n.named_buffers():
                b.copy_(bufs[k])

    def state_dict(self):
        self._ensure_state()
        return {"step": self.step_count, "exp_avg": [self.state[id(n)][0] for n in self.nets],
                "exp_avg_sq": [self.state[id(n)][1] for n in self.nets]}
```

sc-sfmlearner-release_b200/scsfm/nnops.py:

```python
import ctypes

import torch

from . import lib as L

PAD_ZERO, PAD_REFLECT = 0, 1
ACT_NONE, ACT_RELU, ACT_ELU, ACT_DISP = 0, 1, 2, 3
BN_SLOTS = 16
ROUND_TF32 = 0x100
BN_FROZEN = 0x200
OPERAND_TF32, OPERAND_RAW, OPERAND_LO = 0, 1, 2

MODES = ("fp32", "tf32", "tf32x3")


def tune(no_tma=0, mt=0, tw_log2=0, bn=0, wgrad=0):
    t = 1 if no_tma else 0
    t |= (mt & 3) << 4
    t |= ((tw_log2 - 2 if tw_log2 else 0) & 3) << 6
    t |= {0: 0, 16: 1, 32: 2, 64: 3, 128: 4}[bn] << 8
    t |= (wgrad & 3) << 12
    return t


class Conv(ctypes.Structure):
    _fields_ = ([(n, ctypes.c_void_p) for n in ("inp", "w", "bias", "out", "dout", "din", "addend", "dw", "dbias",
                                                "bn_sums")] +
                [(n, ctypes.c_int) for n in ("bn_groups", "B", "Hi", "Wi", "Cin", "Ho", "Wo", "Cout", "kh", "kw",
                                             "stride", "pad", "pad_mode", "act")] +
                [(n, ctypes.c_void_p) for n in ("in_lo", "w_lo", "dout_lo")] +
                [("tune", ctypes.c_uint), ("debug", ctypes.c_void_p)] +
                [(n, ctypes.c_void_p) for n in ("bn_scale", "bn_shift", "out_lo")])


_bound = False


def _lib():
    global _bound
    lib = L.load()
    if not _bound:
        I, P, LL, F = ctypes.c_int, ctypes.c_void_p, ctypes.c_longlong, ctypes.c_float
        CP = ctypes.POINTER(Conv)
        for name in ("scsfm_conv2d_fwd_simt", "scsfm_conv2d_dgrad_simt", "scsfm_conv2d_wgrad_simt",
                     "scsfm_conv2d_fwd_tc", "scsfm_conv2d_dgrad_tc", "scsfm_conv2d_wgrad_tc"):
            getattr(lib, name).argtypes = [CP, P]
        lib.scsfm_round_tf32.argtypes = [P, P, LL, P]
        lib.scsfm_split_tf32.argtypes = [P, P, LL, P]
        lib.scsfm_weight_flip.argtypes = [P, I, I, I, I, P, I, P]
        lib.scsfm_weight_flip_s2.argtypes = [P, I, I, I, I, I, P, I, P]
        lib.scsfm_weight_flip_batched.argtypes = [P, I, I, P]
        lib.scsfm_nchw_to_nhwc.argtypes = [P, P, I, I, I, I, P, P]
        lib.scsfm_nhwc_to_nchw.argtypes = [P, I, I, I, I, P, P]
        lib.scsfm_stem_dgrad.argtypes = [P, P, I, I, I, I, P, P, P]
        lib.scsfm_head_conv_fwd.argtypes = [P, P, P, P, I, I, I, I, I, P]
        lib.scsfm_head_conv_wgrad.argtypes = [P, P, P, P, I, I, I, I, P]
        lib.scsfm_head_conv_dgrad.argtypes = [P, P, P, I, I, I, I, P]
        lib.scsfm_nchw_to_nhwc_pad.argtypes = [P, P, I, I, I, I, I, P, I, P]
        lib.scsfm_pad_channels.argtypes = [P, LL, I, I, P, I, P]
        lib.scsfm_unpad_add.argtypes = [P, LL, I, I, P, P]
        lib.scsfm_bn_prepare.argtypes = [P, I, I, LL, P, P, P, P, F, F, I, P, P]
        lib.scsfm_bn_apply.argtypes = [P, P, P, P, P, P, F, F, P, P, P, P, LL, I, I, I, P]
        lib.scsfm_bn_eval_prepare_batched.argtypes = [P, I, P]
        lib.scsfm_bn_backward.argtypes = [P, P, P, P, P, P, P, P, P, P, LL, I, I, I, P, P]
        lib.scsfm_maxpool_fwd.argtypes = [P, I, I, I, I, P, P, P]
        lib.scsfm_maxpool_bwd.argtypes = [P, P, I, I, I, I, P, I, P]
        lib.scsfm_upcat_fwd.argtypes = [P, P, I, I, I, I, I, P, P]
        lib.scsfm_fold_bwd.argtypes = [P, I, I, I, I, I, I, P, P, I, I, P, P]
        lib.scsfm_act_bwd.argtypes = [P, P, LL, I, P]
        lib.scsfm_spatial_mean_fwd.argtypes = [P, I, I, I, F, P, P]
        lib.scsfm_spatial_mean_bwd.argtypes = [P, I, I, I, F, P, P]
        lib.scsfm_adam_step.argtypes = [P, P, P, P, LL, F, F, F, F, F, I, P, P, I, P]
        _bound = True
    return lib


def round_tf32(src, dst):
    L.launch(_lib().scsfm_round_tf32, "scsfm_round_tf32", "weight_round", 1, 8.0 * src.numel(), L.ptr(src), L.ptr(dst), src.numel(), L.stream())


def split_tf32(src, dst=None):
    if dst is None:
        dst = torch.empty_like(src)
    L.launch(_lib().scsfm_split_tf32, "scsfm_split_tf32", "split", 1, 8.0 * src.numel(), L.ptr(src), L.ptr(dst), src.numel(), L.stream())
    return dst


def lo_of(t):
    lo = getattr(t, "_scsfm_lo", None)
    if lo is None:
        lo = split_tf32(t)
        t._scsfm_lo = lo
    return lo


def empty(shape, like):
    return torch.empty(shape, device=like.device, dtype=torch.float32)


def aligned64(n):
    return (n + 63) // 64 * 64


def tc_supported(kind, Cin, Cout, kh, stride):
    if kind == "fwd":
        return Cin % 4 == 0 and Cout >= 16
    if kind == "dgrad":
        return stride in (1, 2) and Cout % 4 == 0 and Cin >= 16
    if kind == "wgrad":
        return Cin % 4 == 0 and Cout % 4 == 0 and Cout >= 16
    return False


def _s2_classes(kh, kw, pad):
    out = []
    for py in range(2):
        for px in range(2):
            dy_max, dx_max = kh - 1, kw - 1
            while dy_max >= 0 and ((py + pad - dy_max) & 1):
                dy_max -= 1
            while dx_max >= 0 and ((px + pad - dx_max) & 1):
                dx_max -= 1
            jh = 0 if dy_max < 0 else dy_max // 2 + 1
            jw = 0 if dx_max < 0 else dx_max // 2 + 1
            out.append((jh, jw, dy_max, dx_max))
    return out


class FlipTable:

    def __init__(self, cache, device):
        self.keys = sorted(cache)
        rows, blk = [], 0
        for key in self.keys:
            ptr, (Cout, kh, kw, Cin), stride, pad, operand = key
            dst = cache[key][1].data_ptr()
            jobs = [(kh, kw, kh - 1, kw - 1)] if stride == 1 else _s2_classes(kh, kw, pad)
            for (jh, jw, dy_max, dx_max) in jobs:
                total = Cout * jh * jw * Cin
                if total > 0:
                    rows.append([ptr, dst, Cout, kh, kw, Cin, jh, jw, dy_max, dx_max, stride | (operand << 8), blk])
                    blk += ((Cout + 31) // 32) * ((Cin + 31) // 32) * jh * jw
                dst += 4 * total
        self.n_rows, self.total_blocks, self.bytes = len(rows), blk, 8.0 * sum(cache[k][1].numel() for k in self.keys)
        rows.append([0] * 11 + [blk])
        self.table = torch.tensor(rows, dtype=torch.int64).to(device)


def conv_desc(x_shape, w, stride, pad, pad_mode, act):
    B, Hi, Wi, Cin = x_shape
    Cout, kh, kw, _ = w.shape
    Ho = (Hi + 2 * pad - kh) // stride + 1
    Wo = (Wi + 2 * pad - kw) // stride + 1
    return Conv(None, L.ptr(w), None, None, None, None, None, None, None, None, 1, B, Hi, Wi, Cin, Ho, Wo, Cout, kh, kw,
                stride, pad, pad_mode, act, None, None, None, 0, None, None, None, None)


def _tag(d):
    if L.PROF["enabled"]:
        L.TAG["next"] = "B%d %dx%d C%d->%d k%d s%d -> %dx%d" % (d.B, d.Hi, d.Wi, d.Cin, d.Cout, d.kh, d.stride, d.Ho, d.Wo)


def _flops(d):
    return 2.0 * d.B * d.Ho * d.Wo * d.Cout * d.kh * d.kw * d.Cin


class ConvCtx:

    def __init__(self, mode="fp32"):
        if mode not in MODES:
            raise ValueError("conv mode must be one of %s, got %r" % (MODES, mode))
        self.mode = mode
        self.tune = 0
        self.debug = None
        self._flips = {}
        self._table = None
        self.sums_pool = None
        self.wgrad_stream = None
        self._wgrad_keep = []

    @property
    def tc(self):
        return self.mode != "fp32"

    @property
    def split(self):
        return self.mode == "tf32x3"

    def rnd(self):
        return ROUND_TF32 if self.mode == "tf32" else 0

    @property
    def operand(self):
        return OPERAND_TF32 if self.mode == "tf32" else OPERAND_RAW

    def _use_tc(self, kind, Cin, Cout, kh, stride):
        return self.tc and tc_supported(kind, Cin, Cout, kh, stride)

    def _finish(self, d):
        d.tune = self.tune
        d.debug = self.debug.data_ptr() if self.debug is not None else None

    def flipped_weights(self, w, stride, pad, operand):
        key = (w.data_ptr(), tuple(w.shape), stride, pad, operand)
        hit = self._flips.get(key)
        if hit is None:
            Cout, kh, kw, Cin = w.shape
            wt = empty((Cin, kh, kw, Cout), w)
            if stride == 1:
                L.launch(_lib().scsfm_weight_flip, "scsfm_weight_flip", "weight_flip", 1, 8.0 * w.numel(), L.ptr(w), Cout, kh, kw, Cin,
                         L.ptr(wt), operand, L.stream())
            else:
                L.launch(_lib().scsfm_weight_flip_s2, "scsfm_weight_flip_s2", "weight_flip", 4, 8.0 * w.numel(), L.ptr(w), Cout, kh, kw,
                         Cin, pad, L.ptr(wt), operand, L.stream())
            hit = self._flips[key] = (w, wt)
            self._table = None
        return hit[1]

    def refresh_flips(self, device):
        if not self._flips:
            return
        if self._table is None:
            self._table = FlipTable(self._flips, device)
        tab = self._table
        L.launch(_lib().scsfm_weight_flip_batched, "scsfm_weight_flip_batched", "weight_flip", 1, tab.bytes, L.ptr(tab.table), tab.n_rows,
                 tab.total_blocks, L.stream())

    def invalidate(self):
        self._flips.clear()
        self._table = None

    def conv_fwd(self, x, w, bias=None, stride=1, pad=0, pad_mode=PAD_ZERO, act=ACT_NONE, bn_sums=None, bn_groups=1, w_lo=None,
                 bn_scale=None, bn_shift=None, addend=None, with_lo=False):
        lib = _lib()
        d = conv_desc(x.shape, w, stride, pad, pad_mode, act)
        y = empty((d.B, d.Ho, d.Wo, d.Cout), x)
        d.inp, d.bias, d.out, d.bn_sums, d.bn_groups = x.data_ptr(), bias.data_ptr() if bias is not None else None, \
            y.data_ptr(), bn_sums.data_ptr() if bn_sums is not None else None, bn_groups
        if bn_scale is not None:
            d.bn_scale, d.bn_shift = bn_scale.data_ptr(), bn_shift.data_ptr()
        if addend is not None:
            d.addend = addend.data_ptr()
        if with_lo:
            y._scsfm_lo = empty(y.shape, y)
            d.out_lo = y._scsfm_lo.data_ptr()
        tc = self._use_tc("fwd", d.Cin, d.Cout, d.kh, stride)
        if tc and self.split:
            if w_lo is None:
                raise RuntimeError("tf32x3 convolution called without the low part of its weights")
            d.in_lo, d.w_lo = lo_of(x).data_ptr(), w_lo.data_ptr()
        self._finish(d)
        _tag(d)
        fn = lib.scsfm_conv2d_fwd_tc if tc else lib.scsfm_conv2d_fwd_simt
        L.launch(fn, "scsfm_conv2d_fwd", "conv_fwd_tc" if tc else "conv_fwd_simt", 1, _flops(d), ctypes.byref(d), L.stream())
        return y

    def conv_dgrad(self, dout, w, x_shape, stride=1, pad=0, addend=None, padded_input=False, w_src=None):
        lib = _lib()
        B, Hi, Wi, Cin = x_shape
        if padded_input:
            Hi, Wi, pad = Hi + 2, Wi + 2, 0
        d = conv_desc((B, Hi, Wi, Cin), w, stride, pad, PAD_ZERO, ACT_NONE)
        assert (d.Ho, d.Wo, d.Cout) == tuple(dout.shape[1:]), (d.Ho, d.Wo, d.Cout, dout.shape)
        din = empty((B, Hi, Wi, Cin), dout)
        d.dout, d.din, d.addend = dout.data_ptr(), din.data_ptr(), addend.data_ptr() if addend is not None else None
        tc = self._use_tc("dgrad", d.Cin, d.Cout, d.kh, stride)
        if tc:
            if self.split:
                src = w if w_src is None else w_src
                d.w = self.flipped_weights(src, stride, pad, OPERAND_RAW).data_ptr()
                d.w_lo = self.flipped_weights(src, stride, pad, OPERAND_LO).data_ptr()
                d.dout_lo = lo_of(dout).data_ptr()
            else:
                d.w = self.flipped_weights(w, stride, pad, OPERAND_TF32).data_ptr()
        self._finish(d)
        _tag(d)
        fn = lib.scsfm_conv2d_dgrad_tc if tc else lib.scsfm_conv2d_dgrad_simt
        L.launch(fn, "scsfm_conv2d_dgrad", "conv_dgrad_tc" if tc else "conv_dgrad_simt", 1, _flops(d), ctypes.byref(d), L.stream())
        return din

    def conv_wgrad(self, x, dout, dw, dbias=None, stride=1, pad=0, pad_mode=PAD_ZERO):
        lib = _lib()
        d = conv_desc(x.shape, dw, stride, pad, pad_mode, ACT_NONE)
        assert (d.Ho, d.Wo, d.Cout) == tuple(dout.shape[1:])
        d.inp, d.dout, d.dw, d.dbias = x.data_ptr(), dout.data_ptr(), dw.data_ptr(), dbias.data_ptr() if dbias is not None else None
        d.w = None
        tc = self._use_tc("wgrad", d.Cin, d.Cout, d.kh, stride)
        keep = [x, dout]
        if tc and self.split:
            x_lo, dout_lo = lo_of(x), lo_of(dout)
            d.in_lo, d.dout_lo = x_lo.data_ptr(), dout_lo.data_ptr()
            keep += [x_lo, dout_lo]
        self._finish(d)
        _tag(d)
        fn = lib.scsfm_conv2d_wgrad_tc if tc else lib.scsfm_conv2d_wgrad_simt
        with self.on_wgrad_stream(keep):
            L.launch(fn, "scsfm_conv2d_wgrad", "conv_wgrad_tc" if tc else "conv_wgrad_simt", 2 if dbias is not None else 1, _flops(d),
                     ctypes.byref(d), L.stream())

    def on_wgrad_stream(self, keep=()):
        import contextlib
        if self.wgrad_stream is None:
            return contextlib.nullcontext()
        ev = torch.cuda.Event()
        ev.record()
        self.wgrad_stream.wait_event(ev)
        self._wgrad_keep.extend(keep)
        return torch.cuda.stream(self.wgrad_stream)

    def join_wgrad(self):
        if self.wgrad_stream is not None:
            torch.cuda.current_stream().wait_stream(self.wgrad_stream)
        self._wgrad_keep.clear()


def head_fwd(x, w, bias, act):
    B, H, W, C = x.shape
    out = empty((B, H, W, 1), x)
    L.launch(_lib().scsfm_head_conv_fwd, "scsfm_head_conv_fwd", "head_fwd", 1, 4.0 * x.numel(), L.ptr(x), L.ptr(w), L.ptr(bias), L.ptr(out),
             B, H, W, C, act, L.stream())
    return out


def head_dgrad(dpre, w, x_shape):
    B, H, W, C = x_shape
    dpad = empty((B, H + 2, W + 2, C), dpre)
    L.launch(_lib().scsfm_head_conv_dgrad, "scsfm_head_conv_dgrad", "head_dgrad", 1, 4.0 * dpad.numel(), L.ptr(dpre), L.ptr(w), L.ptr(dpad),
             B, H, W, C, L.stream())
    return dpad


def head_wgrad(x, dpre, dw, dbias):
    B, H, W, C = x.shape
    L.launch(_lib().scsfm_head_conv_wgrad, "scsfm_head_conv_wgrad", "head_wgrad", 1, 4.0 * x.numel(), L.ptr(x), L.ptr(dpre), L.ptr(dw),
             L.ptr(dbias), B, H, W, C, L.stream())


def nchw_to_nhwc(a, b=None):
    B, C, H, W = a.shape
    out = empty((B, H, W, C * (2 if b is not None else 1)), a)
    L.launch(_lib().scsfm_nchw_to_nhwc, "scsfm_nchw_to_nhwc", "layout", 1, 8.0 * out.numel(), L.ptr(a), L.ptr(b), B, C, H, W, L.ptr(out), L.stream())
    return out


def nchw_to_nhwc_pad(a, b, Cpad, operand=OPERAND_TF32):
    B, C, H, W = a.shape
    out = empty((B, H, W, Cpad), a)
    L.launch(_lib().scsfm_nchw_to_nhwc_pad, "scsfm_nchw_to_nhwc_pad", "layout", 1, 8.0 * out.numel(), L.ptr(a), L.ptr(b), B, C, H, W, Cpad,
             L.ptr(out), operand, L.stream())
    return out


def pad_channels(w, Cpad, operand=OPERAND_TF32):
    C = w.shape[-1]
    out = empty(tuple(w.shape[:-1]) + (Cpad,), w)
    L.launch(_lib().scsfm_pad_channels, "scsfm_pad_channels", "weight_round", 1, 8.0 * out.numel(), L.ptr(w), w.numel() // C, C, Cpad,
             L.ptr(out), operand, L.stream())
    return out


def unpad_add_(dst, src):
    C, Cpad = dst.shape[-1], src.shape[-1]
    L.launch(_lib().scsfm_unpad_add, "scsfm_unpad_add", "weight_round", 1, 12.0 * dst.numel(), L.ptr(src), dst.numel() // C, C, Cpad,
             L.ptr(dst), L.stream())


def nhwc_to_nchw(x):
    B, H, W, C = x.shape
    out = empty((B, C, H, W), x)
    L.launch(_lib().scsfm_nhwc_to_nchw, "scsfm_nhwc_to_nchw", "layout", 1, 8.0 * out.numel(), L.ptr(x), B, C, H, W, L.ptr(out), L.stream())
    return out


def stem_dgrad(dy, w, H, W, need):
    N, Cin = dy.shape[0], w.shape[-1]
    outs = [empty((N, 3, H, W), dy) if n else None for n in need]
    outs += [None] * (2 - len(outs))
    L.launch(_lib().scsfm_stem_dgrad, "scsfm_stem_dgrad", "stem_dgrad", 1, 2.0 * N * H * W * Cin * 64 * 49 / 4, L.ptr(dy), L.ptr(w),
             N, H, W, Cin, L.ptr(outs[0]), L.ptr(outs[1]), L.stream())
    return outs[:len(need)]


def bn_prepare(sums, groups, count, gamma, beta, rmean, rvar, momentum, eps, training):
    C = gamma.numel()
    saved = empty((groups, C, 4), gamma)
    L.launch(_lib().scsfm_bn_prepare, "scsfm_bn_prepare", "bn_prepare", 1, 0.0, L.ptr(sums), groups, C, count, L.ptr(gamma), L.ptr(beta), L.ptr(rmean), L.ptr(rvar),
                                    momentum, eps, 1 if training else 0, L.ptr(saved), L.stream())
    return saved


def bn_apply(y, sums, gamma, beta, rmean, rvar, momentum, eps, residual, flags, groups=1, with_lo=False):
    z = torch.empty_like(y)
    z_lo = torch.empty_like(y) if with_lo else None
    C = y.shape[-1]
    saved = empty((groups, C, 4), y)
    rows = y.numel() // C
    L.launch(_lib().scsfm_bn_apply, "scsfm_bn_apply", "bn_apply", 1, (12.0 if residual is not None else 8.0) * y.numel(), L.ptr(y), L.ptr(sums),
             L.ptr(gamma), L.ptr(beta), L.ptr(rmean), L.ptr(rvar), momentum, eps, L.ptr(saved), L.ptr(residual), L.ptr(z), L.ptr(z_lo), rows, C,
             groups, int(flags), L.stream())
    if with_lo:
        z._scsfm_lo = z_lo
    return z, saved


class BnEvalTable:

    def __init__(self, bns, eps):
        import struct
        dev = bns[0].weight.device
        total = sum(2 * aligned64(bn.weight.numel()) for bn in bns)
        self.buf = torch.empty(total, device=dev, dtype=torch.float32)
        eps_bits = struct.unpack("<i", struct.pack("<f", eps))[0]
        rows, self.coeffs, off = [], [], 0
        for bn in bns:
            C = bn.weight.numel()
            sc, sh = self.buf[off:off + C], self.buf[off + aligned64(C):off + aligned64(C) + C]
            off += 2 * aligned64(C)
            self.coeffs.append((sc, sh))
            rows.append([bn.weight.data_ptr(), bn.bias.data_ptr(), bn.running_mean.data_ptr(), bn.running_var.data_ptr(),
                         sc.data_ptr(), sh.data_ptr(), C, eps_bits])
        self.key = BnEvalTable.key_of(bns)
        self.table = torch.tensor(rows, dtype=torch.int64).to(dev)
        self.n, self.bytes = len(rows), 24.0 * sum(bn.weight.numel() for bn in bns)

    @staticmethod
    def key_of(bns):
        return tuple((bn.weight.data_ptr(), bn.bias.data_ptr(), bn.running_mean.data_ptr(), bn.running_var.data_ptr()) for bn in bns)

    def prepare(self):
        L.launch(_lib().scsfm_bn_eval_prepare_batched, "scsfm_bn_eval_prepare_batched", "bn_prepare", 1, self.bytes,
                 L.ptr(self.table), self.n, L.stream())


def bn_backward(dz, z, y, saved, dgamma, dbeta, relu, want_dres, groups=1, with_lo=False):
    C = y.shape[-1]
    rows = y.numel() // C
    dy = torch.empty_like(y)
    dy_lo = torch.empty_like(y) if with_lo else None
    work = torch.empty(groups * C * 2, device=y.device, dtype=torch.float64)
    dres = dz if want_dres else None
    frozen = int(relu) & BN_FROZEN
    L.launch(_lib().scsfm_bn_backward, "scsfm_bn_backward", "bn_bwd", 2 if frozen else 4, (20.0 if frozen else 28.0) * y.numel(), L.ptr(dz), L.ptr(z), L.ptr(y), L.ptr(saved), None, L.ptr(dy),
             L.ptr(dy_lo), L.ptr(dres), L.ptr(dgamma), L.ptr(dbeta), rows, C, groups, int(relu), L.ptr(work), L.stream())
    if with_lo:
        dy._scsfm_lo = dy_lo
    return dy, dres


def maxpool_fwd(x):
    B, H, W, C = x.shape
    Ho, Wo = (H - 1) // 2 + 1, (W - 1) // 2 + 1
    y = empty((B, Ho, Wo, C), x)
    idx = torch.empty((B, Ho, Wo, C), device=x.device, dtype=torch.uint8)
    L.launch(_lib().scsfm_maxpool_fwd, "scsfm_maxpool_fwd", "pool", 1, 4.0 * x.numel(), L.ptr(x), B, H, W, C, L.ptr(y), L.ptr(idx), L.stream())
    return y, idx


def maxpool_bwd(dy, idx, x_shape, dx, accumulate):
    B, H, W, C = x_shape
    L.launch(_lib().scsfm_maxpool_bwd, "scsfm_maxpool_bwd", "pool", 1, 4.0 * dx.numel(), L.ptr(dy), L.ptr(idx), B, H, W, C, L.ptr(dx), 1 if accumulate else 0, L.stream())


def upcat_fwd(lo, skip):
    B, h, w, C1 = lo.shape
    C2 = skip.shape[-1] if skip is not None else 0
    out = empty((B, 2 * h, 2 * w, C1 + C2), lo)
    L.launch(_lib().scsfm_upcat_fwd, "scsfm_upcat_fwd", "upcat", 1, 8.0 * out.numel(), L.ptr(lo), L.ptr(skip), B, 2 * h, 2 * w, C1, C2, L.ptr(out), L.stream())
    return out


def fold_plain(dpad, d, act_out, act, accumulate):
    B, Hp, Wp, C = dpad.shape
    L.launch(_lib().scsfm_fold_bwd, "scsfm_fold_bwd", "fold", 1, 8.0 * d.numel(), L.ptr(dpad), B, Hp - 2, Wp - 2, C, 0, 0, L.ptr(d),
             L.ptr(act_out), act, 1 if accumulate else 0, None, L.stream())


def fold_upcat(dpad, C1, lo_act, act):
    B, Hp, Wp, Ct = dpad.shape
    H, W, C2 = Hp - 2, Wp - 2, Ct - C1
    d_lo = empty((B, H // 2, W // 2, C1), dpad)
    d_skip = empty((B, H, W, C2), dpad) if C2 > 0 else None
    L.launch(_lib().scsfm_fold_bwd, "scsfm_fold_bwd", "fold", 2 if C2 > 0 else 1, 4.0 * dpad.numel(), L.ptr(dpad), B, H, W, C1, C2, 1,
             L.ptr(d_lo), L.ptr(lo_act), act, 0, L.ptr(d_skip), L.stream())
    return d_lo, d_skip


def act_bwd_(d, out, act):
    L.launch(_lib().scsfm_act_bwd, "scsfm_act_bwd", "elementwise", 1, 12.0 * d.numel(), L.ptr(d), L.ptr(out), d.numel(), act, L.stream())
    return d


def spatial_mean_fwd(x, scale):
    B, H, W, C = x.shape
    out = empty((B, C), x)
    L.launch(_lib().scsfm_spatial_mean_fwd, "scsfm_spatial_mean_fwd", "pose_head", 1, 4.0 * x.numel(), L.ptr(x), B, H * W, C, scale, L.ptr(out), L.stream())
    return out


def spatial_mean_bwd(dout, x_shape, scale):
    B, H, W, C = x_shape
    dx = empty(x_shape, dout)
    L.launch(_lib().scsfm_spatial_mean_bwd, "scsfm_spatial_mean_bwd", "pose_head", 1, 4.0 * dx.numel(), L.ptr(dout), B, H * W, C, scale, L.ptr(dx), L.stream())
    return dx


def adam_step(param, grad, exp_avg, exp_avg_sq, lr, beta1, beta2, eps, weight_decay, step, step_dev=None, mirror=None,
              mirror_operand=OPERAND_TF32):
    L.launch(_lib().scsfm_adam_step, "scsfm_adam_step", "adam", 1, (32.0 if mirror is not None else 28.0) * param.numel(), L.ptr(param),
             L.ptr(grad), L.ptr(exp_avg), L.ptr(exp_avg_sq), param.numel(), lr, beta1, beta2, eps, weight_decay, step, L.ptr(step_dev),
             L.ptr(mirror), mirror_operand, L.stream())
```

Measured before the change: 77.56.

## Add dedicated warp-specialized TMA stem conv kernel and skip unneeded lo-part tensors

```diff
diff --git a/include/scsfm.h b/include/scsfm.h
--- a/include/scsfm.h
+++ b/include/scsfm.h
@@ -116,6 +116,7 @@
     const float* bn_scale;
     const float* bn_shift;
     float* out_lo;
+    int split;
 } ScsfmConv;
 
 #define SCSFM_TUNE_NO_TMA 0x1u
@@ -131,6 +132,10 @@
 int scsfm_conv2d_fwd_tc(const ScsfmConv* p, void* stream);
 int scsfm_conv2d_dgrad_tc(const ScsfmConv* p, void* stream);
 int scsfm_conv2d_wgrad_tc(const ScsfmConv* p, void* stream);
+#define SCSFM_PASS_FWD 0
+#define SCSFM_PASS_DGRAD 1
+#define SCSFM_PASS_WGRAD 2
+int scsfm_conv_reads_lo(const ScsfmConv* p, int pass);
 #define SCSFM_OPERAND_TF32 0
 #define SCSFM_OPERAND_RAW 1
 #define SCSFM_OPERAND_LO 2
diff --git a/sc-sfmlearner-release_b200/csrc/conv_stem_fwd.cu b/sc-sfmlearner-release_b200/csrc/conv_stem_fwd.cu
--- /dev/null
+++ b/sc-sfmlearner-release_b200/csrc/conv_stem_fwd.cu
@@ -0,0 +1,290 @@
+#include <string.h>
+
+#include "conv_tc.cuh"
+
+namespace scsfm {
+
+constexpr int ST_TH = 8, ST_TW = 16;
+constexpr int ST_ROWS = 2 * ST_TH + 5;
+constexpr int ST_UNITS = ST_TW + 3;
+constexpr int ST_BOX = ST_ROWS * ST_UNITS * 32;
+constexpr int ST_BOX_PITCH = (ST_BOX + 1023) / 1024 * 1024;
+constexpr int ST_THREADS = 384;
+constexpr int ST_PRODUCER_REGS = 40, ST_CONSUMER_REGS = 232;
+constexpr int ST_MAX_STAGES = 8;
+constexpr int ST_SMEM_MAX = 232448;
+
+template <int CIN>
+struct StemCfg {
+    static constexpr int NSL = CIN == 8 ? 7 : 4;
+    static constexpr int NBOX = CIN == 8 ? 2 : 1;
+    static constexpr int KCH = (7 * NSL + 3) / 4;
+    static constexpr int W_BYTES = KCH * 64 * 128;
+    static constexpr int STAGE = NBOX * ST_BOX_PITCH;
+};
+
+struct StemGeom {
+    int tiles_x, tiles_y, num_tiles;
+    int stages;
+};
+
+__device__ __forceinline__ float2 ld_shared_v2(uint32_t saddr) {
+    float2 v;
+    asm volatile("ld.shared.v2.f32 {%0, %1}, [%2];" : "=f"(v.x), "=f"(v.y) : "r"(saddr));
+    return v;
+}
+
+template <int CIN, bool SPLIT>
+__global__ void __launch_bounds__(ST_THREADS, 1)
+conv_stem_fwd_kernel(ScsfmConv p, StemGeom g, const __grid_constant__ CUtensorMap map0, const __grid_constant__ CUtensorMap map1) {
+    using Cfg = StemCfg<CIN>;
+    constexpr int NSL = Cfg::NSL;
+    constexpr int CO = SPLIT ? 32 : 64;
+    constexpr int HALVES = SPLIT ? 2 : 1;
+    extern __shared__ uint8_t smem_raw[];
+    uint8_t* smem = reinterpret_cast<uint8_t*>((reinterpret_cast<uintptr_t>(smem_raw) + 1023) & ~uintptr_t(1023));
+    uint64_t* bar_full = reinterpret_cast<uint64_t*>(smem);
+    uint64_t* bar_empty = bar_full + ST_MAX_STAGES;
+    const uint32_t wsm = tc::smem_u32(smem + 1024);
+    const uint32_t ring = wsm + (uint32_t)Cfg::W_BYTES;
+
+    const int tid = threadIdx.x, warp = tid >> 5, lane = tid & 31;
+    const int n0 = (blockIdx.x % HALVES) * CO;
+    const int t_first = blockIdx.x / HALVES, t_step = gridDim.x / HALVES;
+
+    if (tid == 0) {
+        for (int s = 0; s < g.stages; ++s) {
+            tc::mbar_init(bar_full + s, 1);
+            tc::mbar_init(bar_empty + s, 256);
+        }
+        tc::fence_barrier_init();
+    }
+    for (int i = tid; i < 64 * Cfg::KCH * 32; i += ST_THREADS) {
+        const int n = i / (Cfg::KCH * 32), k = i - n * (Cfg::KCH * 32);
+        const int s = k >> 3, kq = k & 7;
+        const int dy = s / NSL, j = s - dy * NSL;
+        const int word = kq < 4 ? 2 * kq : 2 * kq - 7;
+        const int dx = CIN == 8 ? j : 2 * j + (word >> 2), c = CIN == 8 ? word : (word & 3);
+        float v = 0.f;
+        if (dy < 7 && dx < 7) {
+            const float* src = SPLIT && n >= 32 ? p.w_lo : p.w;
+            const int o = n0 + (SPLIT ? (n & 31) : n);
+            v = __ldg(src + ((o * 7 + dy) * 7 + dx) * CIN + c);
+        }
+        tc::st_shared_f32(wsm + (uint32_t)((k >> 5) * 64 * 128) + tc::sw128_offset(n, k & 31), v);
+    }
+    tc::fence_proxy_async();
+    __syncthreads();
+
+    if (warp >= 8) {
+        tc::setmaxnreg_dec<ST_PRODUCER_REGS>();
+        if (warp == 8 && lane == 0) {
+            tc::tma_prefetch_desc(&map0);
+            if (CIN == 8) tc::tma_prefetch_desc(&map1);
+            int s = 0;
+            uint32_t ph = 0;
+            for (int t = t_first; t < g.num_tiles; t += t_step) {
+                const int tx = t % g.tiles_x, ty = (t / g.tiles_x) % g.tiles_y, b = t / (g.tiles_x * g.tiles_y);
+                const int x0 = tx * ST_TW, iy = 2 * ty * ST_TH - 3;
+                tc::mbar_wait(bar_empty + s, ph ^ 1);
+                const uint32_t st = ring + (uint32_t)(s * Cfg::STAGE);
+                tc::mbar_arrive_expect_tx(bar_full + s, (uint32_t)(Cfg::NBOX * ST_BOX));
+                if (CIN == 8) {
+                    tc::tma_load_4d(st, &map0, 0, x0 - 2, iy, b, bar_full + s);
+                    tc::tma_load_4d(st + ST_BOX_PITCH, &map1, 0, x0 - 1, iy, b, bar_full + s);
+                } else {
+                    tc::tma_load_4d(st, &map0, 0, 2 * x0 - 3, iy, b, bar_full + s);
+                }
+                if (++s == g.stages) { s = 0; ph ^= 1; }
+            }
+        }
+        __syncwarp();
+    } else {
+        tc::setmaxnreg_inc<ST_CONSUMER_REGS>();
+        const int r = warp, gq = lane >> 2, tq = lane & 3;
+        const int groups = p.bn_groups > 0 ? p.bn_groups : 1;
+        const int act = p.act & 0xff;
+        const bool round = (p.act & ROUND_TF32) != 0;
+        float acc[32], part[32];
+        int s = 0;
+        uint32_t ph = 0;
+        for (int t = t_first; t < g.num_tiles; t += t_step) {
+            const int tx = t % g.tiles_x, ty = (t / g.tiles_x) % g.tiles_y, b = t / (g.tiles_x * g.tiles_y);
+            const int x0 = tx * ST_TW, y0 = ty * ST_TH;
+#pragma unroll
+            for (int i = 0; i < 32; ++i) acc[i] = 0.f;
+            tc::mbar_wait(bar_full + s, ph);
+            const uint32_t a_base = ring + (uint32_t)(s * Cfg::STAGE + (2 * r * ST_UNITS + gq) * 32 + 8 * tq);
+#pragma unroll 1
+            for (int dy = 0; dy < 7; ++dy) {
+                uint32_t ahi[NSL][4], alo[NSL][4];
+#pragma unroll
+                for (int j = 0; j < NSL; ++j) {
+                    const int box = CIN == 8 ? (j & 1) : 0, u = CIN == 8 ? (j >> 1) : j;
+                    const uint32_t ad = a_base + (uint32_t)(box * ST_BOX_PITCH + (dy * ST_UNITS + u) * 32);
+                    const float2 v0 = ld_shared_v2(ad), v1 = ld_shared_v2(ad + 8 * 32);
+                    ahi[j][0] = __float_as_uint(v0.x);
+                    ahi[j][1] = __float_as_uint(v1.x);
+                    ahi[j][2] = __float_as_uint(v0.y);
+                    ahi[j][3] = __float_as_uint(v1.y);
+                    if (SPLIT) {
+#pragma unroll
+                        for (int e = 0; e < 4; ++e) alo[j][e] = __float_as_uint(tf32_lo(__uint_as_float(ahi[j][e])));
+                    }
+                }
+                if (dy == 6) tc::mbar_arrive(bar_empty + s);
+                tc::reg_fence(part);
+                tc::wgmma_fence();
+                if (SPLIT) {
+#pragma unroll
+                    for (int j = 0; j < NSL; ++j) {
+                        const int sl = dy * NSL + j;
+                        tc::wgmma_tf32_rs<64>(part, alo[j], tc::make_desc_sw128(wsm + (uint32_t)((sl >> 2) * 64 * 128 + (sl & 3) * 32)),
+                                              j == 0 ? 0u : 1u);
+                    }
+                }
+#pragma unroll
+                for (int j = 0; j < NSL; ++j) {
+                    const int sl = dy * NSL + j;
+                    tc::wgmma_tf32_rs<64>(part, ahi[j], tc::make_desc_sw128(wsm + (uint32_t)((sl >> 2) * 64 * 128 + (sl & 3) * 32)),
+                                          (SPLIT || j > 0) ? 1u : 0u);
+                }
+                tc::wgmma_commit();
+                tc::wgmma_wait<0>();
+                tc::reg_fence(part);
+#pragma unroll
+                for (int i = 0; i < 32; ++i) acc[i] += part[i];
+            }
+            if (++s == g.stages) { s = 0; ph ^= 1; }
+
+            float bs1[CO / 4], bs2[CO / 4];
+#pragma unroll
+            for (int i = 0; i < CO / 4; ++i) { bs1[i] = 0.f; bs2[i] = 0.f; }
+            const int oy = y0 + r;
+#pragma unroll
+            for (int i = 0; i < CO / 8; ++i) {
+                const int c = n0 + 8 * i + 2 * tq;
+                float2 bb = make_float2(0.f, 0.f), sc = make_float2(0.f, 0.f), sh = make_float2(0.f, 0.f);
+                if (p.bias != nullptr) bb = __ldg(reinterpret_cast<const float2*>(p.bias + c));
+                if (p.bn_scale != nullptr) {
+                    sc = __ldg(reinterpret_cast<const float2*>(p.bn_scale + c));
+                    sh = __ldg(reinterpret_cast<const float2*>(p.bn_shift + c));
+                }
+#pragma unroll
+                for (int h = 0; h < 2; ++h) {
+                    const int ox = x0 + gq + 8 * h;
+                    if (oy >= p.Ho || ox >= p.Wo) continue;
+                    float2 x = make_float2(acc[4 * i + 2 * h], acc[4 * i + 2 * h + 1]);
+                    if (SPLIT) { x.x += acc[16 + 4 * i + 2 * h]; x.y += acc[16 + 4 * i + 2 * h + 1]; }
+                    const long long off = (((long long)b * p.Ho + oy) * p.Wo + ox) * 64 + c;
+                    if (p.bias != nullptr) { x.x += bb.x; x.y += bb.y; }
+                    if (p.bn_scale != nullptr) { x.x = fmaf(x.x, sc.x, sh.x); x.y = fmaf(x.y, sc.y, sh.y); }
+                    if (p.addend != nullptr) {
+                        const float2 a = __ldg(reinterpret_cast<const float2*>(p.addend + off));
+                        x.x += a.x; x.y += a.y;
+                    }
+                    if (act != ACT_NONE) { x.x = tc_act(x.x, act); x.y = tc_act(x.y, act); }
+                    if (round) { x.x = tf32_round(x.x); x.y = tf32_round(x.y); }
+                    *reinterpret_cast<float2*>(p.out + off) = x;
+                    if (p.out_lo != nullptr) *reinterpret_cast<float2*>(p.out_lo + off) = make_float2(tf32_lo(x.x), tf32_lo(x.y));
+                    bs1[2 * i] += x.x; bs1[2 * i + 1] += x.y;
+                    bs2[2 * i] += x.x * x.x; bs2[2 * i + 1] += x.y * x.y;
+                }
+            }
+            if (p.bn_sums != nullptr) {
+#pragma unroll
+                for (int o = 4; o < 32; o <<= 1) {
+#pragma unroll
+                    for (int i = 0; i < CO / 4; ++i) {
+                        bs1[i] += __shfl_xor_sync(0xffffffffu, bs1[i], o);
+                        bs2[i] += __shfl_xor_sync(0xffffffffu, bs2[i], o);
+                    }
+                }
+                if (lane < 4) {
+                    const int grp = b / (p.B / groups);
+                    double* d = p.bn_sums + ((size_t)(t % SCSFM_BN_SLOTS) * groups + grp) * 64 * 2;
+#pragma unroll
+                    for (int i = 0; i < CO / 8; ++i) {
+#pragma unroll
+                        for (int e = 0; e < 2; ++e) {
+                            const int c = n0 + 8 * i + 2 * tq + e;
+                            atomicAdd(d + 2 * c, (double)bs1[2 * i + e]);
+                            atomicAdd(d + 2 * c + 1, (double)bs2[2 * i + e]);
+                        }
+                    }
+                }
+            }
+        }
+    }
+}
+
+bool conv_stem_eligible(const ScsfmConv& p) {
+    if (p.tune & SCSFM_TUNE_NO_TMA) return false;
+    if (p.stride != 2 || p.kh != 7 || p.kw != 7 || p.pad != 3 || p.pad_mode != PADMODE_ZERO) return false;
+    if ((p.Cin != 4 && p.Cin != 8) || p.Cout != 64) return false;
+    if (p.Cin == 8 && p.Wi < 2) return false;
+    if (p.in_lo != nullptr && p.w_lo == nullptr) return false;
+    if (p.bn_sums && p.B % (p.bn_groups > 0 ? p.bn_groups : 1) != 0) return false;
+    return true;
+}
+
+static int sm_count() {
+    static int n = 0;
+    if (n == 0) {
+        int dev = 0;
+        if (cudaGetDevice(&dev) != cudaSuccess || cudaDeviceGetAttribute(&n, cudaDevAttrMultiProcessorCount, dev) != cudaSuccess || n <= 0) n = 132;
+    }
+    return n;
+}
+
+static int encode_box(CUtensorMap* m, const float* base, const ScsfmConv& p, int view_cols, int col_step, int box_cols) {
+    const cuuint64_t gdim[4] = {(cuuint64_t)p.Cin, (cuuint64_t)view_cols, (cuuint64_t)p.Hi, (cuuint64_t)p.B};
+    const cuuint64_t gstride[3] = {(cuuint64_t)col_step * p.Cin * 4, (cuuint64_t)p.Wi * p.Cin * 4, (cuuint64_t)p.Hi * p.Wi * p.Cin * 4};
+    const cuuint32_t box[4] = {(cuuint32_t)p.Cin, (cuuint32_t)box_cols, (cuuint32_t)ST_ROWS, 1};
+    const cuuint32_t estr[4] = {1, 1, 1, 1};
+    const CUresult r = encode_tiled(m, CU_TENSOR_MAP_DATA_TYPE_FLOAT32, 4, const_cast<float*>(base), gdim, gstride, box, estr,
+                                    CU_TENSOR_MAP_INTERLEAVE_NONE, CU_TENSOR_MAP_SWIZZLE_NONE, CU_TENSOR_MAP_L2_PROMOTION_L2_256B,
+                                    CU_TENSOR_MAP_FLOAT_OOB_FILL_NONE);
+    if (r != CUDA_SUCCESS) {
+        set_error("cuTensorMapEncodeTiled(stem input %d x %d x %d x %d) failed with CUresult %d", p.B, p.Hi, p.Wi, p.Cin, (int)r);
+        return SCSFM_ERR_CUDA;
+    }
+    return SCSFM_OK;
+}
+
+template <int CIN, bool SPLIT>
+static int launch_stem_cfg(const ScsfmConv& p, cudaStream_t st) {
+    using Cfg = StemCfg<CIN>;
+    static const cudaError_t attr_rc = cudaFuncSetAttribute(conv_stem_fwd_kernel<CIN, SPLIT>, cudaFuncAttributeMaxDynamicSharedMemorySize, ST_SMEM_MAX);
+    SCSFM_CHECK_CUDA(attr_rc);
+    StemGeom g;
+    g.tiles_x = (p.Wo + ST_TW - 1) / ST_TW;
+    g.tiles_y = (p.Ho + ST_TH - 1) / ST_TH;
+    g.num_tiles = g.tiles_x * g.tiles_y * p.B;
+    const int fixed = 1024 + 1024 + Cfg::W_BYTES;
+    g.stages = (ST_SMEM_MAX - fixed) / Cfg::STAGE;
+    if (g.stages > ST_MAX_STAGES) g.stages = ST_MAX_STAGES;
+    CUtensorMap map0, map1;
+    if (CIN == 8) {
+        if (int rc = encode_box(&map0, p.in + CIN, p, p.Wi / 2, 2, ST_UNITS)) return rc;
+        if (int rc = encode_box(&map1, p.in, p, (p.Wi + 1) / 2, 2, ST_UNITS)) return rc;
+    } else {
+        if (int rc = encode_box(&map0, p.in, p, p.Wi, 1, 2 * ST_UNITS)) return rc;
+        map1 = map0;
+    }
+    constexpr int HALVES = SPLIT ? 2 : 1;
+    int ctas = sm_count() / HALVES;
+    if (ctas > g.num_tiles) ctas = g.num_tiles;
+    const size_t smem = (size_t)fixed + (size_t)g.stages * Cfg::STAGE;
+    conv_stem_fwd_kernel<CIN, SPLIT><<<ctas * HALVES, ST_THREADS, smem, st>>>(p, g, map0, map1);
+    SCSFM_CHECK_LAUNCH();
+    return SCSFM_OK;
+}
+
+int launch_conv_stem_fwd(const ScsfmConv& p, cudaStream_t st) {
+    const bool split = p.split || p.w_lo != nullptr;
+    if (p.Cin == 8) return split ? launch_stem_cfg<8, true>(p, st) : launch_stem_cfg<8, false>(p, st);
+    return split ? launch_stem_cfg<4, true>(p, st) : launch_stem_cfg<4, false>(p, st);
+}
+
+}
diff --git a/sc-sfmlearner-release_b200/csrc/conv_tc.cu b/sc-sfmlearner-release_b200/csrc/conv_tc.cu
--- a/sc-sfmlearner-release_b200/csrc/conv_tc.cu
+++ b/sc-sfmlearner-release_b200/csrc/conv_tc.cu
@@ -527,6 +527,33 @@
 
 using namespace scsfm;
 
+static int wgrad_kernel(const ScsfmConv& p) {
+    const bool split = p.split || (p.in_lo != nullptr && p.dout_lo != nullptr);
+    int kernel = (int)((p.tune >> 12) & 3u);
+    if (kernel == 3 && !conv_wgrad_thin_eligible(p)) kernel = 0;
+    if (kernel == 0 && (split || p.in_lo != nullptr || p.dout_lo != nullptr) && conv_wgrad_thin_eligible(p)) kernel = 3;
+    if ((kernel == 0 || kernel == 2) && conv_wgrad_tma_eligible(p) && (split || (p.in_lo == nullptr && p.dout_lo == nullptr))) return 2;
+    return kernel == 3 ? 3 : 1;
+}
+
+static bool conv_reads_lo(const ScsfmConv& p, int pass) {
+    if (pass == SCSFM_PASS_FWD) return !conv_stem_eligible(p);
+    if (pass == SCSFM_PASS_WGRAD) {
+        ScsfmConv q = p;
+        q.split = 1;
+        const int k = wgrad_kernel(q);
+        return k == 1 || (k == 2 && p.pad_mode == PADMODE_REFLECT);
+    }
+    return true;
+}
+
+extern "C" int scsfm_conv_reads_lo(const ScsfmConv* p, int pass) {
+    SCSFM_CHECK_ARG(p != nullptr && pass >= SCSFM_PASS_FWD && pass <= SCSFM_PASS_WGRAD, "conv_reads_lo: bad arguments");
+    SCSFM_CHECK_ARG(p->B > 0 && p->Hi > 0 && p->Wi > 0 && p->Cin > 0 && p->Cout > 0 && p->kh > 0 && p->kw > 0 && p->stride > 0 && p->pad >= 0,
+                    "conv_reads_lo: bad geometry");
+    return conv_reads_lo(*p, pass) ? 1 : 0;
+}
+
 static int tc_dispatch_gather(const ScsfmConv& p, const TcView& v, cudaStream_t st) {
     const int N = p.Cout;
     if (p.in_lo != nullptr && p.w_lo != nullptr && N <= 64) {
@@ -547,6 +574,7 @@
 }
 
 static int tc_dispatch(const ScsfmConv& p, const TcView& v, cudaStream_t st) {
+    if (conv_stem_eligible(p)) return launch_conv_stem_fwd(p, st);
     if (p.pad_mode == PADMODE_ZERO && conv_tma_eligible(p, v) && !s2_prefers_gather(p, v)) return launch_conv_tma(p, v, st);
     if (p.pad_mode == PADMODE_REFLECT && v.in_stride == 1 && p.bn_sums == nullptr && p.Ho >= 3 && p.Wo >= 3 &&
         (p.Ho * p.Wo >= 64 * 208 || conv_tma_forced(p)) && conv_tma_eligible(p, v)) {
@@ -584,6 +612,11 @@
 
 extern "C" int scsfm_conv2d_fwd_tc(const ScsfmConv* p, void* stream) {
     if (int rc = check_tc(p, "conv2d_fwd_tc")) return rc;
+    if (p->split) {
+        SCSFM_CHECK_ARG(p->w_lo != nullptr, "conv2d_fwd_tc: split mode needs w_lo");
+        SCSFM_CHECK_ARG(p->in_lo != nullptr || !conv_reads_lo(*p, SCSFM_PASS_FWD),
+                        "conv2d_fwd_tc: the kernel chosen for this call reads in_lo, which was not passed (scsfm_conv_reads_lo)");
+    }
     return tc_dispatch(*p, plain_view(*p), (cudaStream_t)stream);
 }
 
@@ -666,6 +699,7 @@
 extern "C" int scsfm_conv2d_dgrad_tc(const ScsfmConv* p, void* stream) {
     SCSFM_CHECK_ARG(p != nullptr && p->dout && p->w && p->din, "conv2d_dgrad_tc: null tensor");
     SCSFM_CHECK_ARG(p->stride == 1 || p->stride == 2, "conv2d_dgrad_tc: stride must be 1 or 2");
+    SCSFM_CHECK_ARG(!p->split || (p->dout_lo != nullptr && p->w_lo != nullptr), "conv2d_dgrad_tc: split mode needs dout_lo and w_lo");
     SCSFM_CHECK_ARG(p->kh == p->kw && p->kh - 1 - p->pad >= 0, "conv2d_dgrad_tc: square kernels only");
     cudaStream_t st = (cudaStream_t)stream;
     ScsfmConv q = *p;
@@ -739,13 +773,12 @@
     SCSFM_CHECK_ARG((p->Cin & 3) == 0 && (p->Cout & 3) == 0, "conv2d_wgrad_tc: needs Cin %% 4 == 0 and Cout %% 4 == 0");
     SCSFM_CHECK_ARG(p->pad_mode != PADMODE_REFLECT || p->pad == 1, "conv2d_wgrad_tc: reflect pad must be 1");
     SCSFM_CHECK_ARG((long long)p->B * p->Ho * p->Wo < (1LL << 31), "conv2d_wgrad_tc: too many pixels");
+    SCSFM_CHECK_ARG(!p->split || (p->in_lo != nullptr && p->dout_lo != nullptr) || !conv_reads_lo(*p, SCSFM_PASS_WGRAD),
+                    "conv2d_wgrad_tc: the kernel chosen for this call reads in_lo and dout_lo, which were not passed (scsfm_conv_reads_lo)");
     cudaStream_t st = (cudaStream_t)stream;
     int rc;
-    int kernel = (int)((p->tune >> 12) & 3u);
-    if (kernel == 3 && !conv_wgrad_thin_eligible(*p)) kernel = 0;
-    if (kernel == 0 && (p->in_lo != nullptr || p->dout_lo != nullptr) && conv_wgrad_thin_eligible(*p)) kernel = 3;
-    const bool split = p->in_lo != nullptr && p->dout_lo != nullptr;
-    if ((kernel == 0 || kernel == 2) && conv_wgrad_tma_eligible(*p) && (split || (p->in_lo == nullptr && p->dout_lo == nullptr))) {
+    const int kernel = wgrad_kernel(*p);
+    if (kernel == 2) {
         if ((rc = launch_conv_wgrad_tma(*p, st))) return rc;
         rc = p->pad_mode == PADMODE_REFLECT ? wgrad_gather(*p, 1, st) : SCSFM_OK;
     } else if (kernel == 3) {
diff --git a/sc-sfmlearner-release_b200/csrc/conv_tc.cuh b/sc-sfmlearner-release_b200/csrc/conv_tc.cuh
--- a/sc-sfmlearner-release_b200/csrc/conv_tc.cuh
+++ b/sc-sfmlearner-release_b200/csrc/conv_tc.cuh
@@ -58,6 +58,9 @@
 bool conv_tma_forced(const ScsfmConv& p);
 int launch_conv_tma(const ScsfmConv& p, const TcView& v, cudaStream_t st);
 
+bool conv_stem_eligible(const ScsfmConv& p);
+int launch_conv_stem_fwd(const ScsfmConv& p, cudaStream_t st);
+
 bool conv_wgrad_tma_eligible(const ScsfmConv& p);
 int launch_conv_wgrad_tma(const ScsfmConv& p, cudaStream_t st);
 
diff --git a/sc-sfmlearner-release_b200/csrc/conv_wgrad_tma.cu b/sc-sfmlearner-release_b200/csrc/conv_wgrad_tma.cu
--- a/sc-sfmlearner-release_b200/csrc/conv_wgrad_tma.cu
+++ b/sc-sfmlearner-release_b200/csrc/conv_wgrad_tma.cu
@@ -36,40 +36,6 @@
     uint32_t v;
     asm volatile("ld.shared.b32 %0, [%1];" : "=r"(v) : "r"(saddr));
     return v;
-}
-
-template <int N>
-__device__ __forceinline__ void wgmma_tf32_rs(float (&d)[N / 2], const uint32_t (&a)[4], uint64_t desc_b, uint32_t accumulate);
-template <>
-__device__ __forceinline__ void wgmma_tf32_rs<32>(float (&d)[16], const uint32_t (&a)[4], uint64_t desc_b, uint32_t accumulate) {
-    asm volatile(
-        "{\n\t"
-        ".reg .pred p;\n\t"
-        "setp.ne.b32 p, %21, 0;\n\t"
-        "wgmma.mma_async.sync.aligned.m64n32k8.f32.tf32.tf32 {"
-        "%0, %1, %2, %3, %4, %5, %6, %7, %8, %9, %10, %11, %12, %13, %14, %15"
-        "}, {%16, %17, %18, %19}, %20, p, 1, 1;\n\t"
-        "}\n"
-        : "+f"(d[0]), "+f"(d[1]), "+f"(d[2]), "+f"(d[3]), "+f"(d[4]), "+f"(d[5]), "+f"(d[6]), "+f"(d[7]),
-          "+f"(d[8]), "+f"(d[9]), "+f"(d[10]), "+f"(d[11]), "+f"(d[12]), "+f"(d[13]), "+f"(d[14]), "+f"(d[15])
-        : "r"(a[0]), "r"(a[1]), "r"(a[2]), "r"(a[3]), "l"(desc_b), "r"(accumulate));
-}
-template <>
-__device__ __forceinline__ void wgmma_tf32_rs<64>(float (&d)[32], const uint32_t (&a)[4], uint64_t desc_b, uint32_t accumulate) {
-    asm volatile(
-        "{\n\t"
-        ".reg .pred p;\n\t"
-        "setp.ne.b32 p, %37, 0;\n\t"
-        "wgmma.mma_async.sync.aligned.m64n64k8.f32.tf32.tf32 {"
-        "%0, %1, %2, %3, %4, %5, %6, %7, %8, %9, %10, %11, %12, %13, %14, %15, "
-        "%16, %17, %18, %19, %20, %21, %22, %23, %24, %25, %26, %27, %28, %29, %30, %31"
-        "}, {%32, %33, %34, %35}, %36, p, 1, 1;\n\t"
-        "}\n"
-        : "+f"(d[0]), "+f"(d[1]), "+f"(d[2]), "+f"(d[3]), "+f"(d[4]), "+f"(d[5]), "+f"(d[6]), "+f"(d[7]),
-          "+f"(d[8]), "+f"(d[9]), "+f"(d[10]), "+f"(d[11]), "+f"(d[12]), "+f"(d[13]), "+f"(d[14]), "+f"(d[15]),
-          "+f"(d[16]), "+f"(d[17]), "+f"(d[18]), "+f"(d[19]), "+f"(d[20]), "+f"(d[21]), "+f"(d[22]), "+f"(d[23]),
-          "+f"(d[24]), "+f"(d[25]), "+f"(d[26]), "+f"(d[27]), "+f"(d[28]), "+f"(d[29]), "+f"(d[30]), "+f"(d[31])
-        : "r"(a[0]), "r"(a[1]), "r"(a[2]), "r"(a[3]), "l"(desc_b), "r"(accumulate));
 }
 
 template <int BN, bool SPLIT, int KW, int S>
@@ -223,14 +189,14 @@
                     for (int j = 0; j < NS; ++j) {
                         const int sl = 4 * wg + NS * h + j;
                         const uint32_t boff = (uint32_t)((sl >> 2) * BN * 128 + (sl & 3) * 32);
-                        wgmma_tf32_rs<BN>(part, alo[j], tc::make_desc_sw128(bhi + boff), j == 0 ? 0u : 1u);
-                        wgmma_tf32_rs<BN>(part, ahi[j], tc::make_desc_sw128(blo + boff), 1u);
+                        tc::wgmma_tf32_rs<BN>(part, alo[j], tc::make_desc_sw128(bhi + boff), j == 0 ? 0u : 1u);
+                        tc::wgmma_tf32_rs<BN>(part, ahi[j], tc::make_desc_sw128(blo + boff), 1u);
                     }
 #pragma unroll
                     for (int j = 0; j < NS; ++j) {
                         const int sl = 4 * wg + NS * h + j;
                         const uint32_t boff = (uint32_t)((sl >> 2) * BN * 128 + (sl & 3) * 32);
-                        wgmma_tf32_rs<BN>(part, ahi[j], tc::make_desc_sw128(bhi + boff), 1u);
+                        tc::wgmma_tf32_rs<BN>(part, ahi[j], tc::make_desc_sw128(bhi + boff), 1u);
                     }
                     tc::wgmma_commit();
                     tc::wgmma_wait<0>();
@@ -244,7 +210,7 @@
                     for (int j = 0; j < NS; ++j) {
                         const int sl = 4 * wg + j;
                         const uint32_t boff = (uint32_t)((sl >> 2) * BN * 128 + (sl & 3) * 32);
-                        wgmma_tf32_rs<BN>(acc[dx], ahi[j], tc::make_desc_sw128(bhi + boff), 1u);
+                        tc::wgmma_tf32_rs<BN>(acc[dx], ahi[j], tc::make_desc_sw128(bhi + boff), 1u);
                     }
                     tc::wgmma_commit();
                     tc::wgmma_wait<0>();
@@ -358,7 +324,7 @@
 }
 
 int launch_conv_wgrad_tma(const ScsfmConv& p, cudaStream_t st) {
-    const bool split = p.in_lo != nullptr && p.dout_lo != nullptr;
+    const bool split = p.split || (p.in_lo != nullptr && p.dout_lo != nullptr);
     const unsigned bn_knob = (p.tune >> 8) & 7u;
     const bool bn32 = bn_knob == 2 || (bn_knob != 3 && p.Cout <= 32);
     if (bn32) return split ? launch_wgrad_tma_bn<32, true>(p, st) : launch_wgrad_tma_bn<32, false>(p, st);
diff --git a/sc-sfmlearner-release_b200/csrc/tc_common.cuh b/sc-sfmlearner-release_b200/csrc/tc_common.cuh
--- a/sc-sfmlearner-release_b200/csrc/tc_common.cuh
+++ b/sc-sfmlearner-release_b200/csrc/tc_common.cuh
@@ -146,6 +146,40 @@
         : "l"(desc_a), "l"(desc_b), "r"(accumulate));
 }
 
+template <int N>
+__device__ __forceinline__ void wgmma_tf32_rs(float (&d)[N / 2], const uint32_t (&a)[4], uint64_t desc_b, uint32_t accumulate);
+template <>
+__device__ __forceinline__ void wgmma_tf32_rs<32>(float (&d)[16], const uint32_t (&a)[4], uint64_t desc_b, uint32_t accumulate) {
+    asm volatile(
+        "{\n\t"
+        ".reg .pred p;\n\t"
+        "setp.ne.b32 p, %21, 0;\n\t"
+        "wgmma.mma_async.sync.aligned.m64n32k8.f32.tf32.tf32 {"
+        "%0, %1, %2, %3, %4, %5, %6, %7, %8, %9, %10, %11, %12, %13, %14, %15"
+        "}, {%16, %17, %18, %19}, %20, p, 1, 1;\n\t"
+        "}\n"
+        : "+f"(d[0]), "+f"(d[1]), "+f"(d[2]), "+f"(d[3]), "+f"(d[4]), "+f"(d[5]), "+f"(d[6]), "+f"(d[7]),
+          "+f"(d[8]), "+f"(d[9]), "+f"(d[10]), "+f"(d[11]), "+f"(d[12]), "+f"(d[13]), "+f"(d[14]), "+f"(d[15])
+        : "r"(a[0]), "r"(a[1]), "r"(a[2]), "r"(a[3]), "l"(desc_b), "r"(accumulate));
+}
+template <>
+__device__ __forceinline__ void wgmma_tf32_rs<64>(float (&d)[32], const uint32_t (&a)[4], uint64_t desc_b, uint32_t accumulate) {
+    asm volatile(
+        "{\n\t"
+        ".reg .pred p;\n\t"
+        "setp.ne.b32 p, %37, 0;\n\t"
+        "wgmma.mma_async.sync.aligned.m64n64k8.f32.tf32.tf32 {"
+        "%0, %1, %2, %3, %4, %5, %6, %7, %8, %9, %10, %11, %12, %13, %14, %15, "
+        "%16, %17, %18, %19, %20, %21, %22, %23, %24, %25, %26, %27, %28, %29, %30, %31"
+        "}, {%32, %33, %34, %35}, %36, p, 1, 1;\n\t"
+        "}\n"
+        : "+f"(d[0]), "+f"(d[1]), "+f"(d[2]), "+f"(d[3]), "+f"(d[4]), "+f"(d[5]), "+f"(d[6]), "+f"(d[7]),
+          "+f"(d[8]), "+f"(d[9]), "+f"(d[10]), "+f"(d[11]), "+f"(d[12]), "+f"(d[13]), "+f"(d[14]), "+f"(d[15]),
+          "+f"(d[16]), "+f"(d[17]), "+f"(d[18]), "+f"(d[19]), "+f"(d[20]), "+f"(d[21]), "+f"(d[22]), "+f"(d[23]),
+          "+f"(d[24]), "+f"(d[25]), "+f"(d[26]), "+f"(d[27]), "+f"(d[28]), "+f"(d[29]), "+f"(d[30]), "+f"(d[31])
+        : "r"(a[0]), "r"(a[1]), "r"(a[2]), "r"(a[3]), "l"(desc_b), "r"(accumulate));
+}
+
 __device__ __forceinline__ uint64_t make_desc_sw128(uint32_t saddr) {
     uint64_t d = 0;
     d |= (uint64_t)((saddr >> 4) & 0x3FFF);
diff --git a/sc-sfmlearner-release_b200/scsfm/nets.py b/sc-sfmlearner-release_b200/scsfm/nets.py
--- a/sc-sfmlearner-release_b200/scsfm/nets.py
+++ b/sc-sfmlearner-release_b200/scsfm/nets.py
@@ -521,8 +521,9 @@
     else:
         d_f0 = torch.empty_like(f0)
         O.maxpool_bwd(d, rec["pool_idx"], f0.shape, d_f0, False)
+    w_shape = (t.conv1.weight.shape[0], t.conv1.k, t.conv1.k, x.shape[-1])
     dy, _ = O.bn_backward(d_f0, f0, stem.y, stem.saved, *_bn_param_grads(t.bn1, plan), 1 | cx.rnd() | plan.bn, False, G,
-                          cx.split and plan.params)
+                          plan.params and cx.wgrad_reads_lo(x.shape, w_shape, 2, 3))
     if plan.params:
         if x.shape[-1] != t.conv1.weight.shape[1]:
             dw = torch.zeros(t.conv1.weight.shape[0], t.conv1.k, t.conv1.k, x.shape[-1], device=x.device, dtype=torch.float32)
diff --git a/sc-sfmlearner-release_b200/scsfm/nnops.py b/sc-sfmlearner-release_b200/scsfm/nnops.py
--- a/sc-sfmlearner-release_b200/scsfm/nnops.py
+++ b/sc-sfmlearner-release_b200/scsfm/nnops.py
@@ -30,7 +30,10 @@
                                              "stride", "pad", "pad_mode", "act")] +
                 [(n, ctypes.c_void_p) for n in ("in_lo", "w_lo", "dout_lo")] +
                 [("tune", ctypes.c_uint), ("debug", ctypes.c_void_p)] +
-                [(n, ctypes.c_void_p) for n in ("bn_scale", "bn_shift", "out_lo")])
+                [(n, ctypes.c_void_p) for n in ("bn_scale", "bn_shift", "out_lo")] +
+                [("split", ctypes.c_int)])
+
+PASS_FWD, PASS_DGRAD, PASS_WGRAD = 0, 1, 2
 
 
 _bound = False
@@ -45,6 +48,7 @@
         for name in ("scsfm_conv2d_fwd_simt", "scsfm_conv2d_dgrad_simt", "scsfm_conv2d_wgrad_simt",
                      "scsfm_conv2d_fwd_tc", "scsfm_conv2d_dgrad_tc", "scsfm_conv2d_wgrad_tc"):
             getattr(lib, name).argtypes = [CP, P]
+        lib.scsfm_conv_reads_lo.argtypes = [CP, I]
         lib.scsfm_round_tf32.argtypes = [P, P, LL, P]
         lib.scsfm_split_tf32.argtypes = [P, P, LL, P]
         lib.scsfm_weight_flip.argtypes = [P, I, I, I, I, P, I, P]
@@ -149,7 +153,8 @@
 
 def conv_desc(x_shape, w, stride, pad, pad_mode, act):
     B, Hi, Wi, Cin = x_shape
-    Cout, kh, kw, _ = w.shape
+    Cout, kh, kw, _ = w if isinstance(w, tuple) else w.shape
+    w = None if isinstance(w, tuple) else w
     Ho = (Hi + 2 * pad - kh) // stride + 1
     Wo = (Wi + 2 * pad - kw) // stride + 1
     return Conv(None, L.ptr(w), None, None, None, None, None, None, None, None, 1, B, Hi, Wi, Cin, Ho, Wo, Cout, kh, kw,
@@ -200,6 +205,18 @@
     def _finish(self, d):
         d.tune = self.tune
         d.debug = self.debug.data_ptr() if self.debug is not None else None
+
+    def _reads_lo(self, d, pass_):
+        rc = _lib().scsfm_conv_reads_lo(ctypes.byref(d), pass_)
+        L.check(0 if rc >= 0 else rc, "scsfm_conv_reads_lo")
+        return rc == 1
+
+    def wgrad_reads_lo(self, x_shape, w_shape, stride, pad, pad_mode=PAD_ZERO):
+        if not (self.split and self._use_tc("wgrad", x_shape[-1], w_shape[0], w_shape[1], stride)):
+            return False
+        d = conv_desc(tuple(x_shape), tuple(w_shape), stride, pad, pad_mode, ACT_NONE)
+        self._finish(d)
+        return self._reads_lo(d, PASS_WGRAD)
 
     def flipped_weights(self, w, stride, pad, operand):
         key = (w.data_ptr(), tuple(w.shape), stride, pad, operand)
@@ -248,8 +265,10 @@
         if tc and self.split:
             if w_lo is None:
                 raise RuntimeError("tf32x3 convolution called without the low part of its weights")
-            d.in_lo, d.w_lo = lo_of(x).data_ptr(), w_lo.data_ptr()
+            d.w_lo, d.split = w_lo.data_ptr(), 1
         self._finish(d)
+        if tc and self.split and self._reads_lo(d, PASS_FWD):
+            d.in_lo = lo_of(x).data_ptr()
         _tag(d)
         fn = lib.scsfm_conv2d_fwd_tc if tc else lib.scsfm_conv2d_fwd_simt
         L.launch(fn, "scsfm_conv2d_fwd", "conv_fwd_tc" if tc else "conv_fwd_simt", 1, _flops(d), ctypes.byref(d), L.stream())
@@ -270,7 +289,7 @@
                 src = w if w_src is None else w_src
                 d.w = self.flipped_weights(src, stride, pad, OPERAND_RAW).data_ptr()
                 d.w_lo = self.flipped_weights(src, stride, pad, OPERAND_LO).data_ptr()
-                d.dout_lo = lo_of(dout).data_ptr()
+                d.dout_lo, d.split = lo_of(dout).data_ptr(), 1
             else:
                 d.w = self.flipped_weights(w, stride, pad, OPERAND_TF32).data_ptr()
         self._finish(d)
@@ -287,11 +306,13 @@
         d.w = None
         tc = self._use_tc("wgrad", d.Cin, d.Cout, d.kh, stride)
         keep = [x, dout]
+        self._finish(d)
         if tc and self.split:
-            x_lo, dout_lo = lo_of(x), lo_of(dout)
-            d.in_lo, d.dout_lo = x_lo.data_ptr(), dout_lo.data_ptr()
-            keep += [x_lo, dout_lo]
-        self._finish(d)
+            d.split = 1
+            if self._reads_lo(d, PASS_WGRAD):
+                x_lo, dout_lo = lo_of(x), lo_of(dout)
+                d.in_lo, d.dout_lo = x_lo.data_ptr(), dout_lo.data_ptr()
+                keep += [x_lo, dout_lo]
         _tag(d)
         fn = lib.scsfm_conv2d_wgrad_tc if tc else lib.scsfm_conv2d_wgrad_simt
         with self.on_wgrad_stream(keep):
```

Result: faster. 83.25 (median of 6 runs) (+7.3%).
